# gpcv-liujin/Ada-MVS

Hardware: AMD Instinct MI355X
Metric: depth maps/sec at 768x384x5-view x192-hyp (hot path, features resident in HBM) (higher is better)
Workload: dtype f32; 1 GPU; cfg2: 5 views, 768x384, hypotheses 192, fp32; concurrent_tile_groups=1, parallelism=tile-sharded x1, 1 RCCL gather per step, launch=hipGraph replay

## Files before the change

### ada-mvs_amd/csrc/api.hip

```cpp
#include <stdarg.h>
#include <string.h>

#include <atomic>
#include <mutex>

#include "../../include/adamvs_hip.h"
#include "common.h"
#include "kernels.h"

namespace adamvs {

thread_local char g_last_error[512] = "";

int set_error(int code, const char* fmt, ...) {
  va_list ap;
  va_start(ap, fmt);
  vsnprintf(g_last_error, sizeof(g_last_error), fmt, ap);
  va_end(ap);
  return code;
}

static_assert(sizeof(FuseWeights) == sizeof(adamvs_fuse_weights), "adamvs_fuse_weights layout");

struct OptionEntry { const char* name; int def; };
// ... 86 lines not shown
    size_t F = (size_t)s.S * s.B * hw * stage_reg_width(s);
    c.sim = take(F);
    c.score = take(F);
    c.creg = take(3 * F);
  }
  c.total = o;
  return c;
}

static int check_desc(const adamvs_stage_desc* d) {
  ADAMVS_CHECK_ARG(d, "stage: null descriptor");
  ADAMVS_CHECK_ARG(d->B > 0 && d->S > 0 && d->D > 1 && d->h > 1 && d->w > 1, "stage: bad shape (B=%d S=%d D=%d h=%d w=%d)",
                   d->B, d->S, d->D, d->h, d->w);
  ADAMVS_CHECK_ARG(d->C == 8 || d->C == 16 || d->C == 32, "stage: C=%d unsupported (8, 16 or 32)", d->C);
  ADAMVS_CHECK_ARG((d->h % 2) == 0 && (d->w % 2) == 0, "stage: h=%d w=%d must be even", d->h, d->w);
  ADAMVS_CHECK_ARG(d->B <= 65535, "stage: B=%d tiles per call (at most 65535)", d->B);
  ADAMVS_CHECK_ARG(d->precision == PRECISION_FP32 || d->precision == PRECISION_BF16X3, "stage: precision=%d (0 fp32, 1 bf16x3)", d->precision);
  ADAMVS_CHECK_ARG(d->eps_in_numerator == 0 || d->eps_in_numerator == 1, "stage: eps_in_numerator=%d (0 or 1)", d->eps_in_numerator);
  ADAMVS_CHECK_ARG(d->plane_mode >= PLANES_EXPLICIT && d->plane_mode <= PLANES_WINDOW, "stage: plane_mode=%d (0 explicit, 1 uniform, 2 window)", d->plane_mode);
  ADAMVS_CHECK_ARG(d->precision_fuse == PRECISION_FP32 || d->precision_fuse == PRECISION_BF16X3,
                   "stage: precision_fuse=%d (0 fp32, 1 bf16x3)", d->precision_fuse);
  if (d->first_stage) {
    ADAMVS_CHECK_ARG(stage_reg_width(*d) > 0, "stage: D=%d hypotheses: CostRegNet2D runs at widths up to 512", d->D);
    ADAMVS_CHECK_ARG((d->h % 8) == 0 && (d->w % 8) == 0, "stage: first stage needs h=%d w=%d multiples of 8", d->h, d->w);
  } else {
    ADAMVS_CHECK_ARG(d->prev_h > 0 && d->prev_w > 0, "stage: prev_h/prev_w missing");
  }
  return 0;
}

}

using namespace adamvs;

extern "C" int adamvs_version(void) { return ADAMVS_ABI_VERSION; }

extern "C" int adamvs_option_count(void) { return OPT_COUNT; }
extern "C" const char* adamvs_option_name(int index) { return index >= 0 && index < OPT_COUNT ? g_option_table[index].name : nullptr; }
extern "C" int adamvs_option_default(const char* name, int* value) {
  const int i = option_index(name);
  ADAMVS_CHECK_ARG(i >= 0 && value, "option_default: unknown option '%s' (include/adamvs_hip.h, OPTIONS)", name ? name : "(null)");
  *value = g_option_table[i].def;
  return 0;
}
extern "C" int adamvs_get_option(const char* name, int* value) {
  const int i = option_index(name);
  ADAMVS_CHECK_ARG(i >= 0 && value, "get_option: unknown option '%s' (include/adamvs_hip.h, OPTIONS)", name ? name : "(null)");
  *value = opt((Option)i);
  return 0;
}
extern "C" int adamvs_set_option(const char* name, int value) {
  const int i = option_index(name);
  ADAMVS_CHECK_ARG(i >= 0, "set_option: unknown option '%s' (include/adamvs_hip.h, OPTIONS)", name ? name : "(null)");
  option_init();
  g_option_value[i].store(value, std::memory_order_relaxed);
  return 0;
}
extern "C" const char* adamvs_last_error_string(void) { return g_last_error; }

extern "C" size_t adamvs_slice_reg_step_scratch_bytes(int B, int h, int w) {
  size_t hw = (size_t)h * w, hw4 = (size_t)(h / 2) * (w / 2);
  return (3 * align_up((size_t)B * hw * 8) + 3 * align_up((size_t)B * hw4 * 16)) * sizeof(float);
}

extern "C" int adamvs_slice_reg_step(const float* cost, float* state1, float* state2, const adamvs_fuse_weights* weights,
                                     float* reg_cost, int B, int C, int h, int w, int in_up, int precision, void* scratch,
                                     size_t scratch_bytes, void* stream) {
  ADAMVS_CHECK_ARG(precision == PRECISION_FP32 || precision == PRECISION_BF16X3, "slice_reg_step: precision=%d (0 fp32, 1 bf16x3)", precision);
  ADAMVS_CHECK_ARG(cost && state1 && state2 && weights && reg_cost && scratch, "slice_reg_step: null pointer");
  ADAMVS_CHECK_ARG(B > 0 && h > 1 && w > 1 && (h % 2) == 0 && (w % 2) == 0, "slice_reg_step: bad shape (B=%d h=%d w=%d, even sizes)", B, h, w);
  ADAMVS_CHECK_ARG(C == 8 || C == 16 || C == 32, "slice_reg_step: C=%d unsupported (8, 16 or 32)", C);
  ADAMVS_CHECK_ARG(scratch_bytes >= adamvs_slice_reg_step_scratch_bytes(B, h, w), "slice_reg_step: scratch too small");
  hipStream_t st = (hipStream_t)stream;
  size_t n1 = align_up((size_t)B * h * w * 8), n2 = align_up((size_t)B * (h / 2) * (w / 2) * 16);
  float* s = (float*)scratch;
  float* c1 = s;
  StepBuffers sb{state1, s + n1, s + 2 * n1, s + 3 * n1, state2, s + 3 * n1 + n2, s + 3 * n1 + 2 * n2};
  FuseWeights fw;
  memcpy(&fw, weights, sizeof(fw));
  int rc = launch_conv1(cost, fw.conv1, c1, B, C, h, w, precision, st);
  if (rc) return rc;
  float* h1_now = state1;
  float* h2_now = state2;
  if ((rc = launch_slice_step(c1, fw, sb, reg_cost, B, h, w, 1, 0, in_up, precision, st, &h1_now, &h2_now))) return rc;
  if (h1_now != state1) {
    hipError_t e = copy_floats(h1_now, state1, (size_t)B * h * w * 8, st);
    if (e != hipSuccess) return set_error((int)e, "slice_reg_step: state copy: %s", hipGetErrorString(e));
  }
  if (h2_now != state2) {
    hipError_t e = copy_floats(h2_now, state2, (size_t)B * (h / 2) * (w / 2) * 16, st);
    if (e != hipSuccess) return set_error((int)e, "slice_reg_step: state copy: %s", hipGetErrorString(e));
  }
  return 0;
}

extern "C" int adamvs_recurrence_schedule(int precision_fuse, long long pixels) { return recurrence_mode(precision_fuse, (long)pixels); }
extern "C" int adamvs_gru_wino_mask(void) { return gru_wino_mask(); }

extern "C" size_t adamvs_depth_stage_workspace_bytes(const adamvs_stage_desc* desc) {
  if (check_desc(desc)) return 0;
  return carve(*desc).total * sizeof(float);
}

static int stage_forward(const adamvs_stage_desc* desc, const float* feat, const float* rt, const float* planes,
                         const float* prev_conf, const float* w_reg, size_t w_reg_floats, const adamvs_fuse_weights* w_fuse,
                         float* view_weight, float* pair_depth, float* depth, float* confidence, int phases, void* workspace,
                         size_t workspace_bytes, void* stream, bool timing_only) {
  int rc = check_desc(desc);
  if (rc) return rc;
  ADAMVS_CHECK_ARG(phases >= 0 && phases <= ADAMVS_PHASE_ALL, "stage: phases=%d (a subset of ADAMVS_PHASE_ALL = 15)", phases);
  const adamvs_stage_desc& s = *desc;
  ADAMVS_CHECK_ARG(feat && rt && planes && w_fuse && view_weight && depth && confidence && workspace, "stage: null pointer");
  ADAMVS_CHECK_ARG(!s.first_stage || (w_reg && pair_depth), "stage: first stage needs w_reg and pair_depth");
  ADAMVS_CHECK_ARG(!s.first_stage || w_reg_floats == cost_reg_weight_floats(stage_reg_width(s), s.precision),
                   "stage: w_reg holds %zu floats; D=%d hypotheses run at width %d, whose layout has %zu (include/adamvs_hip.h)",
                   w_reg_floats, s.D, stage_reg_width(s), cost_reg_weight_floats(stage_reg_width(s), s.precision));
  ADAMVS_CHECK_ARG(s.first_stage || prev_conf, "stage: later stages need prev_conf");
  StageCarve c = carve(s);
  ADAMVS_CHECK_ARG(workspace_bytes >= c.total * sizeof(float), "stage: workspace too small (%zu < %zu bytes)", workspace_bytes,
                   c.total * sizeof(float));
  hipStream_t st = (hipStream_t)stream;
  float* ws = (float*)workspace;
  FuseWeights fw;
  memcpy(&fw, w_fuse, sizeof(fw));
  const PlaneSrc ps{planes, s.plane_mode, s.half_span, s.plane_mode == PLANES_WINDOW ? s.half_span_dev : nullptr};

  if (!(phases & ADAMVS_PHASE_VIEW_WEIGHTS)) {
  } else if (s.first_stage) {
    const int Dr = stage_reg_width(s);
    if ((rc = launch_pair_similarity(feat, rt, ps, ws + c.sim, s.B, s.S, s.C, s.D, s.h, s.w, st, Dr))) return rc;
    if (cost_reg_softmax_fusable(Dr, s.precision, ps)) {
      if ((rc = launch_cost_reg_net_2d(ws + c.sim, w_reg, ws + c.creg, ws + c.score, s.S * s.B, Dr, s.h, s.w, s.precision, st,
                                       view_weight, pair_depth, &ps, s.B, s.D)))
        return rc;
    } else {
      if ((rc = launch_cost_reg_net_2d(ws + c.sim, w_reg, ws + c.creg, ws + c.score, s.S * s.B, Dr, s.h, s.w, s.precision, st))) return rc;
      if ((rc = launch_softmax_regress(ws + c.score, ps, view_weight, pair_depth, s.S, s.B, Dr, s.h, s.w, st, s.D))) return rc;
    }
  } else {
    if ((rc = adamvs_resize_bilinear(prev_conf, view_weight, s.S * s.B, s.prev_h, s.prev_w, s.h, s.w, stream))) return rc;
  }

  const bool do_agg = phases & ADAMVS_PHASE_AGGREGATE, do_rec = phases & ADAMVS_PHASE_RECURRENCE, do_arg = phases & ADAMVS_PHASE_SOFT_ARGMIN;
  if (!do_agg && !do_rec && !do_arg) return 0;
  const size_t hw = (size_t)s.h * s.w, hw4 = (size_t)(s.h / 2) * (s.w / 2);
  const int dc = c.dc, nchunks = (s.D + dc - 1) / dc;
  ADAMVS_CHECK_ARG(nchunks == 1 || (do_agg && do_rec && do_arg) || timing_only,
                   "stage: phases=%d selects a proper subset of AGGREGATE|RECURRENCE|SOFT_ARGMIN, but D=%d runs in %d chunks of %d "
                   "hypotheses and the workspace keeps one: pass all three in one call (adamvs_bench_stage_phase times one "
                   "phase alone, no maps)", phases, s.D, nchunks, dc);
  const size_t c1_stride = (size_t)s.B * hw * 8;
  GruStateRing rb{{ws + c.h1[0], ws + c.h1[1], ws + c.h1[2], ws + c.h1[3]}, ws + c.rh1, ws + c.u1, {ws + c.c2[0], ws + c.c2[1]},
                  {ws + c.h2[0], ws + c.h2[1]}, ws + c.rh2, ws + c.u2};
  const int mode = recurrence_mode(s.precision_fuse, (long)s.B * s.h * s.w);
  const bool pipelined = mode != 0;
  const int lag = recurrence_lags(mode, s.precision_fuse).dec;
  if (do_rec) {
    hipError_t e = zero_floats(pipelined ? rb.h1[3] : rb.h1[0], (size_t)s.B * hw * 8, st);
    if (e == hipSuccess) e = zero_floats(pipelined ? rb.h2[1] : rb.h2[0], (size_t)s.B * hw4 * 16, st);
    if (e != hipSuccess) return set_error((int)e, "stage: zero initial states: %s", hipGetErrorString(e));
  }
  auto vol_of = [&](int d) { return ws + c.vol[(d / dc) & 1]; };
  auto argmin_chunk = [&](int k) {
    const int d0 = k * dc, nd = (d0 + dc < s.D ? d0 + dc : s.D) - d0;
    return launch_soft_argmin_chunk(ws + c.vol[k & 1], dc, ps, s.D, d0, nd, ws + c.acc, k == 0, k == nchunks - 1, depth, confidence,
                                    s.B, s.h, s.w, s.in_up, st);
  };
  StepBuffers sb{rb.h1[0], rb.rh1, rb.u1, rb.c2[0], rb.h2[0], rb.rh2, rb.u2};
  for (int k = 0; k < nchunks; ++k) {
    const int d0 = k * dc, d1 = d0 + dc < s.D ? d0 + dc : s.D;
    if (do_agg && (rc = launch_sweep_conv1_chunk(feat, rt, ps, view_weight, fw.conv1, ws + c.c1, ws + c.agg, s.B, s.S, s.C, s.D, d0,
                                                 d1, s.h, s.w, s.precision_fuse, s.eps_in_numerator, st)))
      return rc;
    if (do_rec) {
      for (int t = d0; t < d1; ++t) {
        const float* c1_t = ws + c.c1 + (size_t)(t - d0) * c1_stride;
        if (pipelined) {
          const int sd = t - lag;
          if ((rc = launch_recur_pipeline_step(rb, fw, s.B, s.h, s.w, s.D, t, c1_t, sd >= 0 ? vol_of(sd) : nullptr, dc, sd >= 0 ? sd % dc : 0,
                                               s.in_up, s.precision_fuse, mode, st)))
            return rc;
          if (do_arg && sd >= 0 && sd % dc == dc - 1 && (rc = argmin_chunk(sd / dc))) return rc;
        } else if ((rc = launch_slice_step(c1_t, fw, sb, vol_of(t), s.B, s.h, s.w, dc, t % dc, s.in_up, s.precision_fuse, st))) {
          return rc;
        }
      }
      if (!pipelined && do_arg && (rc = argmin_chunk(k))) return rc;
    } else if (do_arg && (rc = argmin_chunk(k))) {
      return rc;
    }
  }
  if (do_rec && pipelined) {
    for (int t = s.D; t < s.D + lag; ++t) {
      const int sd = t - lag;
      if ((rc = launch_recur_pipeline_step(rb, fw, s.B, s.h, s.w, s.D, t, nullptr, sd >= 0 ? vol_of(sd) : nullptr, dc, sd >= 0 ? sd % dc : 0,
                                           s.in_up, s.precision_fuse, mode, st)))
        return rc;
      if (do_arg && sd >= 0 && sd % dc == dc - 1 && sd / dc < nchunks - 1 && (rc = argmin_chunk(sd / dc))) return rc;
    }
    if (do_arg && (rc = argmin_chunk(nchunks - 1))) return rc;
  }
  return 0;
}

extern "C" int adamvs_depth_stage_forward(const adamvs_stage_desc* desc, const float* feat, const float* rt,
                                          const float* planes, const float* prev_conf, const float* w_reg, size_t w_reg_floats,
                                          const adamvs_fuse_weights* w_fuse, float* view_weight, float* pair_depth,
                                          float* depth, float* confidence, int phases, void* workspace,
                                          size_t workspace_bytes, void* stream) {
  return stage_forward(desc, feat, rt, planes, prev_conf, w_reg, w_reg_floats, w_fuse, view_weight, pair_depth, depth, confidence,
                       phases, workspace, workspace_bytes, stream, false);
}

extern "C" int adamvs_bench_stage_phase(const adamvs_stage_desc* desc, const float* feat, const float* rt,
                                        const float* planes, const float* prev_conf, const float* w_reg, size_t w_reg_floats,
                                        const adamvs_fuse_weights* w_fuse, float* view_weight, float* pair_depth,
                                        float* depth, float* confidence, int phases, void* workspace,
                                        size_t workspace_bytes, void* stream) {
  return stage_forward(desc, feat, rt, planes, prev_conf, w_reg, w_reg_floats, w_fuse, view_weight, pair_depth, depth, confidence,
                       phases, workspace, workspace_bytes, stream, true);
}

extern "C" int adamvs_fusion_max_sources(void) { return ADAMVS_FUSION_MAX_SOURCES; }

static bool finite_f(float v) { return v == v && v <= 3.402823466e38f && v >= -3.402823466e38f; }

extern "C" int adamvs_geo_consistency(const float* ref_depth, const float* ref_conf, int H, int W, const adamvs_fusion_source* sources,
                                      int N, float prob_threshold, float pix_threshold, float rel_depth_threshold, int min_consistent,
                                      unsigned char* count, float* fused, unsigned* block_kept, void* stream) {
  ADAMVS_CHECK_ARG(ref_depth && ref_conf && sources && count && fused && block_kept, "geo_consistency: null pointer");
  ADAMVS_CHECK_ARG(H > 0 && W > 0 && (long)H * W < (1L << 31), "geo_consistency: bad reference size H=%d W=%d", H, W);
  ADAMVS_CHECK_ARG(N >= 1 && N <= ADAMVS_FUSION_MAX_SOURCES, "geo_consistency: N=%d sources (1 .. %d)", N, ADAMVS_FUSION_MAX_SOURCES);
  ADAMVS_CHECK_ARG(finite_f(prob_threshold), "geo_consistency: prob_threshold is not finite");
  ADAMVS_CHECK_ARG(finite_f(pix_threshold) && pix_threshold > 0.f, "geo_consistency: pix_threshold must be finite and > 0");
  ADAMVS_CHECK_ARG(finite_f(rel_depth_threshold) && rel_depth_threshold > 0.f, "geo_consistency: rel_depth_threshold must be finite and > 0");
  ADAMVS_CHECK_ARG(min_consistent >= 0, "geo_consistency: min_consistent=%d (>= 0)", min_consistent);
  for (int s = 0; s < N; ++s) {
    ADAMVS_CHECK_ARG(sources[s].depth, "geo_consistency: source %d: null depth pointer", s);
    ADAMVS_CHECK_ARG(sources[s].H > 0 && sources[s].W > 0 && (long)sources[s].H * sources[s].W < (1L << 31),
                     "geo_consistency: source %d: bad size H=%d W=%d", s, sources[s].H, sources[s].W);
    for (int k = 0; k < 12; ++k)
      ADAMVS_CHECK_ARG(finite_f(sources[s].fwd[k]) && finite_f(sources[s].back[k]), "geo_consistency: source %d: transform not finite", s);
  }
  return launch_geo_consistency(ref_depth, ref_conf, H, W, sources, N, prob_threshold, pix_threshold, rel_depth_threshold, min_consistent,
                                count, fused, block_kept, (hipStream_t)stream);
}

extern "C" int adamvs_fusion_scan(const unsigned* block_kept, unsigned* offsets, int nblocks, void* stream) {
  ADAMVS_CHECK_ARG(block_kept && offsets, "fusion_scan: null pointer");
  ADAMVS_CHECK_ARG(nblocks > 0, "fusion_scan: nblocks=%d (> 0)", nblocks);
  return launch_fusion_scan(block_kept, offsets, nblocks, (hipStream_t)stream);
}

extern "C" int adamvs_fusion_emit(const float* fused, const unsigned char* rgba, int H, int W, const double* camera, const unsigned* offsets,
                                  double* xyz, unsigned char* rgb, long capacity, void* stream) {
  ADAMVS_CHECK_ARG(fused && rgba && camera && offsets && xyz && rgb, "fusion_emit: null pointer");
  ADAMVS_CHECK_ARG(H > 0 && W > 0 && (long)H * W < (1L << 31), "fusion_emit: bad size H=%d W=%d", H, W);
  ADAMVS_CHECK_ARG(capacity >= (long)H * W, "fusion_emit: capacity %ld < H W = %ld points", capacity, (long)H * W);
  for (int k = 0; k < 21; ++k)
    ADAMVS_CHECK_ARG(std::isfinite(camera[k]), "fusion_emit: camera[%d] is not finite", k);
  return launch_fusion_emit(fused, rgba, H, W, camera, offsets, xyz, rgb, capacity, (hipStream_t)stream);
}

static int dsm_check_grid(const adamvs_dsm_grid* g, const char* what) {
  ADAMVS_CHECK_ARG(g, "%s: null grid", what);
  ADAMVS_CHECK_ARG(std::isfinite(g->gsd) && g->gsd > 0.0, "%s: gsd=%g must be finite and > 0", what, g->gsd);
  ADAMVS_CHECK_ARG(std::isfinite(g->x0) && std::isfinite(g->y_top) && std::isfinite(g->z_ref), "%s: grid origin / z_ref not finite", what);
  ADAMVS_CHECK_ARG(g->W > 0 && g->H > 0 && (long)g->W * g->H <= ADAMVS_DSM_MAX_CELLS, "%s: grid W=%d H=%d (W H <= %d cells)", what, g->W,
                   g->H, ADAMVS_DSM_MAX_CELLS);
  return 0;
}

static int dsm_check_points(long n, long seq0, const char* what) {
  ADAMVS_CHECK_ARG(n >= 0, "%s: n=%ld (>= 0)", what, n);
  ADAMVS_CHECK_ARG(seq0 >= 0 && seq0 <= (1L << 32) - n, "%s: seq0=%ld + n=%ld exceeds 2^32 points", what, seq0, n);
  return 0;
}

extern "C" int adamvs_dsm_accumulate(const adamvs_dsm_grid* grid, const double* xyz, long n, long seq0, int mode, unsigned long long* key,
                                     unsigned* count, long long* sum, void* stream) {
  if (int rc = dsm_check_grid(grid, "dsm_accumulate")) return rc;
  if (int rc = dsm_check_points(n, seq0, "dsm_accumulate")) return rc;
  ADAMVS_CHECK_ARG(mode == ADAMVS_DSM_MAX || mode == ADAMVS_DSM_MEAN, "dsm_accumulate: mode=%d (0 max, 1 mean)", mode);
  ADAMVS_CHECK_ARG(xyz && key && count && (sum || mode == ADAMVS_DSM_MAX), "dsm_accumulate: null pointer");
  return launch_dsm_accumulate(*grid, xyz, n, seq0, mode, key, count, sum, (hipStream_t)stream);
}

extern "C" int adamvs_dsm_claim(const adamvs_dsm_grid* grid, const double* xyz, const unsigned char* rgb, long n, long seq0,
                                const unsigned long long* key, unsigned* color, void* stream) {
  if (int rc = dsm_check_grid(grid, "dsm_claim")) return rc;
  if (int rc = dsm_check_points(n, seq0, "dsm_claim")) return rc;
  ADAMVS_CHECK_ARG(xyz && rgb && key && color, "dsm_claim: null pointer");
  return launch_dsm_claim(*grid, xyz, rgb, n, seq0, key, color, (hipStream_t)stream);
}

extern "C" int adamvs_dsm_finalize(const adamvs_dsm_grid* grid, const unsigned long long* key, const unsigned* count, const long long* sum,
                                   const unsigned* color, int mode, int min_count, float* dsm, unsigned short* count16, unsigned char* rgba,
                                   void* stream) {
  if (int rc = dsm_check_grid(grid, "dsm_finalize")) return rc;
  ADAMVS_CHECK_ARG(mode == ADAMVS_DSM_MAX || mode == ADAMVS_DSM_MEAN, "dsm_finalize: mode=%d (0 max, 1 mean)", mode);
  ADAMVS_CHECK_ARG(min_count >= 1, "dsm_finalize: min_count=%d (>= 1)", min_count);
  ADAMVS_CHECK_ARG(key && count && color && dsm && count16 && rgba && (sum || mode == ADAMVS_DSM_MAX), "dsm_finalize: null pointer");
  return launch_dsm_finalize(*grid, key, count, sum, color, mode, min_count, dsm, count16, (unsigned*)rgba, (hipStream_t)stream);
}

static int dsm_fill_check_size(int W, int H, const char* what) {
  ADAMVS_CHECK_ARG(W > 0 && H > 0 && (long)W * H <= ADAMVS_DSM_MAX_CELLS, "%s: grid W=%d H=%d (W H <= %d cells)", what, W, H,
// ... 658 lines not shown
```

### ada-mvs_amd/csrc/kernels.h

```cpp
#pragma once
#include <stdlib.h>

#include "common.h"
#include "options.h"
#include "planes.h"
#include "../../include/adamvs_hip.h"

namespace adamvs {

enum { PRECISION_FP32 = 0, PRECISION_BF16X3 = 1 };

hipError_t zero_floats(float* p, size_t n, hipStream_t st);
hipError_t copy_floats(const float* src, float* dst, size_t n, hipStream_t st);

struct FuseWeights {
  const float* conv1;
  const float* gates1; const float* gates1_b;
  const float* cand1;  const float* cand1_b;
  const float* conv2;
  const float* gates2; const float* gates2_b;
  const float* cand2;  const float* cand2_b;
  const float* upconv1; const float* upconv1_b;
  const float* final_w;
  const float* gates1_w; const float* gates2_w; const float* cand2_w; const float* cand1_w;
};
int gru_wino_mask();

struct StepBuffers {
  float* h1; float* rh1; float* u1;
  float* c2; float* h2; float* rh2; float* u2;
};

struct GruStateRing {
  float* h1[4]; float* rh1; float* u1;
  float* c2[2]; float* h2[2]; float* rh2; float* u2;
};
struct RecurLags { int c2, dec; };
int recurrence_mode(int precision, long pixels);
RecurLags recurrence_lags(int schedule, int precision);
int launch_recur_pipeline_step(const GruStateRing& rb, const FuseWeights& fw, int B, int h, int w, int D, int t, const float* c1_t,
                               float* vol_dec, int D_vol, int d_dec, int in_up, int precision, int schedule, hipStream_t st);
int launch_soft_argmin_chunk(const float* vol, int vol_D, PlaneSrc planes, int D, int d0, int nd, float* acc, int first, int last,
                             float* depth, float* conf, int B, int h, int w, int in_up, hipStream_t st);
int sweep_chunk_planes(int D);
int launch_sweep_conv1_chunk(const float* feat, const float* rt, PlaneSrc planes, const float* vw, const float* w1pk,
                             float* c1_chunk, float* sim_ws, int B, int S, int C, int D, int d0, int d1, int h, int w, int precision,
                             int eps_in_numerator, hipStream_t st);

int launch_conv1(const float* cost, const float* w, float* c1, int B, int C, int h, int w_, int precision, hipStream_t st);
int launch_conv1_bf16x3(const float* cost, const float* w, float* c1, int N, int C, int h, int w_, hipStream_t st);
int launch_gru_convs_bf16x3(const float* c1, const FuseWeights& fw, const StepBuffers& sb, int B, int h, int w, int d,
                            float** h1_now, float** h2_now, hipStream_t st);
int launch_slice_step(const float* c1, const FuseWeights& fw, const StepBuffers& sb, float* vol, int B, int h, int w, int D,
                      int d, int in_up, int precision, hipStream_t st, float** h1_now = nullptr, float** h2_now = nullptr);
enum { GRU_PRO_NONE = 0, GRU_PRO_GATES = 1, GRU_PRO_OUT = 2 };
struct GruPro {
  int mode;
  const float* f;
  const float* o;
  const double* part_f;
  const double* part_o;
  int parts_f, group_f, parts_o;
  const float* gn_f;
  const float* gn_o;
  float* state_out;
  float* R; int RW;
  int hc, count;
  float eps;
};

constexpr int GN_PARTS_LIMIT = 2048;
inline bool gn_epilogue_partials(long parts, int samples) { return parts > 0 && parts <= GN_PARTS_LIMIT && parts * samples <= 4096; }
int launch_conv_pair(const float* srcA, int CA, const float* srcB, int CB, const float* wpk, const float* bias, float* out,
                     int cout, int B, int h, int w, hipStream_t st, double* gn_part = nullptr, int gn_hc = 0, int gn_groups = 0,
                     int* gn_parts = nullptr, const GruPro* pro = nullptr);
bool conv_pair_epilogue_partials(int B, int h, int w);
inline bool gru_fold_enabled(int samples) {
  const int forced = opt(OPT_RED_FOLD_APPLIES);
  return forced >= 0 ? forced != 0 : samples <= 2;
}
bool can_fold_gru_applies(int N, int D, int h, int w);
int launch_conv_dd_gates_gn(const float* in, const float* wpk_r, const float* bias_r, const float* skip_r, float* out_r,
                            const float* wpk_u, const float* bias_u, const float* skip_u, float* out_u, int N, int D, int h, int w,
                            hipStream_t st, double* gn_part, int gn_n, int* gn_parts, const GruPro* pro = nullptr);
int launch_conv_dd_gn(const float* in, const float* wpk, const float* bias, const float* skip, float* out, int N, int D, int h, int w,
                      hipStream_t st, double* gn_part, int gn_n, int gn_group, int gn_ngroups, int* gn_parts, const GruPro* pro = nullptr);
int launch_soft_argmin(const float* vol, const float* planes, float* depth, float* conf, int B, int D, int h, int w,
                       int in_up, hipStream_t st);
int launch_sweep_conv1(const float* feat, const float* rt, PlaneSrc planes, const float* vw, const float* w1pk,
                       float* c1, float* sim_ws, int B, int S, int C, int D, int h, int w, int precision, int eps_in_numerator,
                       hipStream_t st);
int launch_sweep_variance(const float* feat, const float* rt, const float* planes, float* out_a, int Da, float* out_b, int Db,
                          int B, int S, int C, int D, int h, int w, hipStream_t st);
size_t sweep_workspace_floats(int B, int C, int D, int h, int w);
int launch_cost_reg_net_2d(const float* x, const float* wpk, float* ws, float* score, int N, int D, int h, int w,
                           int precision, hipStream_t st, float* sm_vw = nullptr, float* sm_pd = nullptr,
                           const PlaneSrc* sm_planes = nullptr, int sm_B = 1, int n_planes = 0);
size_t cost_reg_weight_floats(int D, int precision);
int costreg_width(int D);
int costreg_width_bf16x3(int D);
bool cost_reg_softmax_fusable(int D, int precision, const PlaneSrc& planes);
int launch_conv_dd_bf16x3(const float* in, const float* wpk, const float* bias, const float* skip, float* out, int N, int D,
                          int hi, int wi, int ho, int wo, int mode, int relu, hipStream_t st, float* sm_vw = nullptr,
                          float* sm_pd = nullptr, const PlaneSrc* sm_planes = nullptr, int sm_B = 1, int n_planes = 0);
bool costreg_bf16x3_depth_supported(int D);
bool wino_depth_supported(int D);
bool cost_reg_winograd(int D, int precision);
bool wino_softmax_fused();
size_t wino_softmax_part_floats(int N, int D, int h, int w);
int launch_conv_wino_softmax(const float* in, const float* wpk, const float* bias, float* part, const PlaneSrc& planes, float* vw, float* pd,
                             int N, int B, int D, int n_planes, int h, int w, hipStream_t st);
int launch_conv_wino(const float* in, const float* wpk, const float* bias, const float* skip, float* out, int N, int D, int h, int w,
                     int relu, hipStream_t st);

int launch_pair_similarity(const float* feat, const float* rt, PlaneSrc planes, float* sim, int B, int S, int C, int D, int h,
                           int w, hipStream_t st, int Dw = 0);
int launch_softmax_regress(const float* score, PlaneSrc planes, float* vw, float* pd, int S, int B, int D, int h, int w,
                           hipStream_t st, int n_planes = 0);
bool costreg_depth_supported(int D);

constexpr int FUSION_TILE = ADAMVS_FUSION_TILE;
constexpr int FUSION_MAX_SOURCES = ADAMVS_FUSION_MAX_SOURCES;
int launch_geo_consistency(const float* ref_depth, const float* ref_conf, int H, int W, const adamvs_fusion_source* srcs, int N,
                           float prob_threshold, float pix_threshold, float rel_depth_threshold, int min_consistent, uint8_t* count,
                           float* fused, unsigned* block_kept, hipStream_t st);
int launch_fusion_scan(const unsigned* counts, unsigned* offsets, int nblocks, hipStream_t st);
int launch_fusion_emit(const float* fused, const uint8_t* rgba, int H, int W, const double* camera, const unsigned* offsets, double* xyz,
                       uint8_t* rgb, long capacity, hipStream_t st);

constexpr int DSM_TILE = 256;
int launch_dsm_accumulate(const adamvs_dsm_grid& g, const double* xyz, long n, long seq0, int mode, unsigned long long* key,
                          unsigned* count, long long* sum, hipStream_t st);
int launch_dsm_claim(const adamvs_dsm_grid& g, const double* xyz, const uint8_t* rgb, long n, long seq0, const unsigned long long* key,
                     unsigned* color, hipStream_t st);
int launch_dsm_finalize(const adamvs_dsm_grid& g, const unsigned long long* key, const unsigned* count, const long long* sum,
                        const unsigned* color, int mode, int min_count, float* dsm, uint16_t* count16, unsigned* rgba, hipStream_t st);

long dsm_fill_workspace_bytes(int W, int H);
int launch_dsm_fill(int W, int H, const float* dsm, const uint8_t* rgba, double r_cells, double tol_height, double tol_colour,
                    int max_cycles, void* workspace, float* dsm_out, uint8_t* rgba_out, int* dist2, uint8_t* filled,
                    adamvs_dsm_fill_stats* stats, hipStream_t st);

constexpr int MESH_TILE = ADAMVS_MESH_TILE;
int launch_tsdf_integrate(const adamvs_mesh_brick& b, const adamvs_mesh_view* views, int nviews, const int* list, int nlist, float* tsdf,
                          uint16_t* weight, unsigned* rgba, hipStream_t st);
int launch_mesh_classify(const adamvs_mesh_brick& b, const float* tsdf, const uint16_t* weight, unsigned* cube_code, unsigned* block_tris,
                         hipStream_t st);
int launch_mesh_count_vertices(const adamvs_mesh_brick& b, const float* tsdf, const unsigned* cube_code, uint8_t* edge_mask,
                               unsigned* block_verts, hipStream_t st);
int launch_mesh_emit(const adamvs_mesh_brick& b, const float* tsdf, const unsigned* rgba, const unsigned* cube_code, const uint8_t* edge_mask,
                     const unsigned* vert_offsets, const unsigned* tri_offsets, unsigned vertex_base, double* xyz, uint8_t* rgb,
                     unsigned* first_vertex, long vert_capacity, unsigned* faces, long tri_capacity, hipStream_t st);

constexpr int SIMPLIFY_TILE = ADAMVS_SIMPLIFY_TILE;
int launch_simplify_keys(const double* origin, double cell, const double* xyz, long nv, long long* keys, uint8_t* bad, hipStream_t st);
int launch_simplify_corners(const unsigned* faces, long nf, const int* vcell, long nv, int nc, int* fcell, int* entry_cell, uint8_t* survive,
                            hipStream_t st);
int launch_simplify_accumulate(const double* origin, double cell, const long long* keys, int nc, const double* xyz, const uint8_t* rgb,
                               long nv, const unsigned* faces, long nf, const long long* entry, const long long* fstart,
                               const long long* vorder, const long long* vstart, double* quadric, double* member,
                               unsigned long long* colour, hipStream_t st);
int launch_simplify_solve(const double* origin, double cell, double rank_eps, const long long* keys, int nc, const double* quadric,
                          const double* member, const unsigned long long* colour, const long long* vstart, double* pos, uint8_t* col,
                          uint8_t* rank, uint8_t* fallback, double* error, hipStream_t st);
void simplify_solve_host(const double* quadric, const double* mean, double cell, double rank_eps, double* p, int* rank, int* fallback,
                         double* error);
int launch_simplify_triples(const int* fcell, long nf, const long long* surv, long ns, int* tri, hipStream_t st);
int launch_simplify_first(const int* tri, const long long* surv, const long long* order, long ns, long nf, uint8_t* keep, hipStream_t st);
int launch_simplify_mark(const int* fcell, const uint8_t* keep, long nf, int nc, uint8_t* used, hipStream_t st);
int launch_simplify_count(const uint8_t* flags, long n, unsigned* block_count, hipStream_t st);
int launch_simplify_emit(const double* pos, const uint8_t* col, const uint8_t* used, int nc, const unsigned* cell_offsets, const int* fcell,
                         const uint8_t* keep, long nf, const unsigned* face_offsets, double* xyz, uint8_t* rgb, unsigned* new_index,
                         long vert_capacity, unsigned* faces, long face_capacity, hipStream_t st);

constexpr int SMOOTH_TILE = ADAMVS_SMOOTH_TILE;
int launch_smooth_faces(const double* p, long nv, const unsigned* faces, long nf, double* rec, hipStream_t st);
int launch_mesh_edge_keys(const unsigned* faces, long nf, long long* keys, const char* what, hipStream_t st);
int launch_smooth_boundary(const long long* keys, long n, long nv, uint8_t* fixed, hipStream_t st);
int launch_smooth_filter(const double* rec, const double* nin, double* nout, const unsigned* faces, long nf, long nv, const int* vface,
                         const long long* vstart, double sigma_s, double sigma_r, hipStream_t st);
int launch_smooth_centroids(const double* p, long nv, const unsigned* faces, long nf, double* cen, hipStream_t st);
int launch_smooth_update(const double* p0, const double* p, double* pout, long nv, const double* nrm, const double* cen, long nf,
                         const int* vface, const long long* vstart, const uint8_t* fixed, double cap, uint8_t* clamped, hipStream_t st);

constexpr int CLEAN_TILE = ADAMVS_CLEAN_TILE;
constexpr int CLEAN_CHUNK = ADAMVS_CLEAN_CHUNK;
int launch_clean_components(const unsigned* faces, long nf, long nv, const int* parent_in, int* parent_out, unsigned* changed, hipStream_t st);
int launch_clean_area(const double* area, long nf, const long long* order, const long long* seg_of, const long long* seg_start, long ncomp,
                      double* lead, double* first, double* out, hipStream_t st);
int launch_clean_boundary(const long long* keys, const long long* entry, long n, uint8_t* bnd, hipStream_t st);
int launch_clean_successor(const unsigned* faces, long ns, long nv, const uint8_t* bnd, int* out_cnt, int* in_cnt, int* out_he, int* succ,
                           int* lab, int* nxt, uint8_t* broken, hipStream_t st);
int launch_clean_double(const uint8_t* bnd, long n, const int* lab_in, const int* nxt_in, const uint8_t* broken_in, int* lab_out, int* nxt_out,
                        uint8_t* broken_out, hipStream_t st);
// ... 76 lines not shown
```

### ada-mvs_amd/csrc/options.h

```cpp
#pragma once

namespace adamvs {

#define ADAMVS_OPTION_LIST(X)                                                                                                     \
  X(OPT_WINOGRAD, "winograd", 1)                      \
  X(OPT_WINO_SOFTMAX, "wino_softmax", 1)                              \
  X(OPT_WINO_WPS, "wino_wps", 0)                                                   \
  X(OPT_FUSE_SOFTMAX, "fuse_softmax", 1)                        \
  X(OPT_S2_PAIRS, "s2_pairs", 1)                            \
  X(OPT_CONV_ROWS2, "conv_rows2", -1)                               \
  X(OPT_T2_FUSED, "t2_fused", -1)                                  \
  X(OPT_T2_KB8, "t2_kb8", 1)                                                 \
  X(OPT_COSTREG_DEFER_SKIPS, "costreg_defer_skips", 1)                            \
  X(OPT_CONV256_SPLIT, "conv256_split", 1)                                          \
  X(OPT_CONV_SMALL_GRID, "conv_small_grid", 1024)         \
  X(OPT_RED_FOLD_APPLIES, "red_fold_applies", -1)               \
  X(OPT_CONV1_F23, "conv1_f23", 3)                             \
  X(OPT_FCONV_F23, "fconv_f23", 1)                                \
  X(OPT_GRU_WINO, "gru_wino", 7)                      \
  X(OPT_RECUR_MODE, "recur_mode", -1)

enum Option {
#define ADAMVS_OPTION_ENUM(e, n, d) e,
  ADAMVS_OPTION_LIST(ADAMVS_OPTION_ENUM)
#undef ADAMVS_OPTION_ENUM
  OPT_COUNT
};

int opt(Option o);

}
```

### ada-mvs_amd/csrc/recurrence.hip

```cpp
#include <stdlib.h>

#include "common.h"
#include "kernels.h"
#include "persistent.h"
#include "slice_roles.h"
#include "slice_roles_bx3.h"
#include "slice_roles_fused.h"
#include "slice_roles_wino.h"

namespace adamvs {

struct NopRole {
  struct Args {};
  static constexpr size_t LDS_BYTES = 0;
  static int tiles_x(const Args&) { return 1; }
  static int tiles_y(const Args&) { return 1; }
  static __device__ __forceinline__ void run(const Args&, const TileGrid&, TileRange, int, int, float*) {}
};

template <class R0, class R1, class R2>
struct SlotArgs {
  typename R0::Args a0; TileGrid g0; TileRange r0; int n0;
  typename R1::Args a1; TileGrid g1; TileRange r1; int n1;
  typename R2::Args a2; TileGrid g2; TileRange r2;
};

template <class R> struct min_blocks { static constexpr int value = 1; };
template <> struct min_blocks<Gru1FusedBx3Role> { static constexpr int value = 2; };
template <> struct min_blocks<Gru2FusedBx3Role> { static constexpr int value = 2; };
template <> struct min_blocks<Gru2FusedRole<4>> { static constexpr int value = 2; };
template <> struct min_blocks<ConvWinoRole<16, 16, 2, EPI_GATES>> { static constexpr int value = 2; };
constexpr int imax3(int a, int b, int c) { return a > b ? (a > c ? a : c) : (b > c ? b : c); }

template <class R0, class R1, class R2>
__global__ __launch_bounds__(256, imax3(min_blocks<R0>::value, min_blocks<R1>::value, min_blocks<R2>::value)) void k_slot(SlotArgs<R0, R1, R2> s) {
  extern __shared__ __attribute__((aligned(16))) float lds[];
  const int wg = blockIdx.x;
  if (wg < s.n0) R0::run(s.a0, s.g0, s.r0, wg, s.n0, lds);
  else if (wg < s.n0 + s.n1) R1::run(s.a1, s.g1, s.r1, wg - s.n0, s.n1, lds);
  else R2::run(s.a2, s.g2, s.r2, wg - s.n0 - s.n1, (int)gridDim.x - s.n0 - s.n1, lds);
}

constexpr size_t max3(size_t a, size_t b, size_t c) { return a > b ? (a > c ? a : c) : (b > c ? b : c); }

template <class R>
struct RoleUse {
  const typename R::Args* args;
  float cost;
  float f0, f1;
};

template <int NR>
static void split_grid(int total, const long (&tiles)[NR], const double (&work)[NR], int (&n)[NR]) {
  double W = 0;
  for (int i = 0; i < NR; ++i) W += tiles[i] ? work[i] : 0;
  int sum = 0;
  for (int i = 0; i < NR; ++i) {
    n[i] = 0;
    if (!tiles[i]) continue;
    long v = (long)(total * (work[i] / W) + 0.5);
    n[i] = (int)(v < 1 ? 1 : (v > tiles[i] ? tiles[i] : v));
    sum += n[i];
  }
  while (sum > total) {
    int k = -1;
    for (int i = 0; i < NR; ++i) if (n[i] > 1 && (k < 0 || n[i] > n[k])) k = i;
    if (k < 0) break;
    --n[k]; --sum;
  }
  while (sum < total) {
    int k = -1;
    for (int i = 0; i < NR; ++i)
      if (tiles[i] && n[i] < tiles[i] && (k < 0 || work[i] / n[i] > work[k] / n[k])) k = i;
    if (k < 0) break;
    ++n[k]; ++sum;
  }
}

template <class R0, class R1, class R2>
static int launch_slot(const RoleUse<R0>& u0, const RoleUse<R1>& u1, const RoleUse<R2>& u2, int B, hipStream_t st, const char* name) {
  constexpr size_t lds = max3(R0::LDS_BYTES, R1::LDS_BYTES, R2::LDS_BYTES);
  static_assert(lds <= 160 * 1024, "slot exceeds the LDS of a CU");
  constexpr auto kern = k_slot<R0, R1, R2>;
  int capacity, rc;
  if ((rc = resident_capacity<kern>(lds, name, &capacity))) return rc;
  SlotArgs<R0, R1, R2> s;
  memset(&s, 0, sizeof(s));
  long tiles[3] = {0, 0, 0};
  double work[3] = {0, 0, 0};
  auto prep = [&](auto* args, auto& dst_args, TileGrid& g, TileRange& r, float cost, float f0, float f1, int i, auto role) -> int {
    typedef decltype(role) R;
    if (!args) return 0;
    dst_args = *args;
    if (int e = make_tile_grid(g, R::tiles_x(*args), R::tiles_y(*args), B)) return e;
    r.begin = (int)((double)g.ntiles * f0 + 0.5);
    r.end = f1 >= 1.0f ? g.ntiles : (int)((double)g.ntiles * f1 + 0.5);
    tiles[i] = r.end - r.begin;
    work[i] = (double)tiles[i] * cost;
    return 0;
  };
  if ((rc = prep(u0.args, s.a0, s.g0, s.r0, u0.cost, u0.f0, u0.f1, 0, R0()))) return rc;
  if ((rc = prep(u1.args, s.a1, s.g1, s.r1, u1.cost, u1.f0, u1.f1, 1, R1()))) return rc;
  if ((rc = prep(u2.args, s.a2, s.g2, s.r2, u2.cost, u2.f0, u2.f1, 2, R2()))) return rc;
  const long all = tiles[0] + tiles[1] + tiles[2];
  if (all == 0) return 0;
  int n[3];
  split_grid<3>((int)(all < capacity ? all : capacity), tiles, work, n);
  s.n0 = n[0];
  s.n1 = n[1];
  hipLaunchKernelGGL(kern, dim3(n[0] + n[1] + n[2]), dim3(256), lds, st, s);
  ADAMVS_CHECK_LAUNCH(name);
  return 0;
}

template <class R0, class R1, class R2, class R3>
struct SlotArgs4 {
  typename R0::Args a0; TileGrid g0; TileRange r0; int n0;
  typename R1::Args a1; TileGrid g1; TileRange r1; int n1;
  typename R2::Args a2; TileGrid g2; TileRange r2; int n2;
  typename R3::Args a3; TileGrid g3; TileRange r3;
};
constexpr int imax4(int a, int b, int c, int d) { return imax3(imax3(a, b, c), d, d); }
constexpr size_t max4(size_t a, size_t b, size_t c, size_t d) { return max3(max3(a, b, c), d, d); }

template <class R0, class R1, class R2, class R3>
__global__ __launch_bounds__(256, imax4(min_blocks<R0>::value, min_blocks<R1>::value, min_blocks<R2>::value, min_blocks<R3>::value))
void k_slot4(SlotArgs4<R0, R1, R2, R3> s) {
  extern __shared__ __attribute__((aligned(16))) float lds[];
  const int wg = blockIdx.x;
  if (wg < s.n0) R0::run(s.a0, s.g0, s.r0, wg, s.n0, lds);
  else if (wg < s.n0 + s.n1) R1::run(s.a1, s.g1, s.r1, wg - s.n0, s.n1, lds);
  else if (wg < s.n0 + s.n1 + s.n2) R2::run(s.a2, s.g2, s.r2, wg - s.n0 - s.n1, s.n2, lds);
  else R3::run(s.a3, s.g3, s.r3, wg - s.n0 - s.n1 - s.n2, (int)gridDim.x - s.n0 - s.n1 - s.n2, lds);
}

template <class R0, class R1, class R2, class R3>
static int launch_slot4(const RoleUse<R0>& u0, const RoleUse<R1>& u1, const RoleUse<R2>& u2, const RoleUse<R3>& u3, int B, hipStream_t st,
                        const char* name) {
  constexpr size_t lds = max4(R0::LDS_BYTES, R1::LDS_BYTES, R2::LDS_BYTES, R3::LDS_BYTES);
  static_assert(lds <= 64 * 1024, "slot exceeds the default dynamic LDS limit");
  constexpr auto kern = k_slot4<R0, R1, R2, R3>;
  int capacity, rc;
  if ((rc = resident_capacity<kern>(lds, name, &capacity))) return rc;
  SlotArgs4<R0, R1, R2, R3> s;
  memset(&s, 0, sizeof(s));
  long tiles[4] = {0, 0, 0, 0};
  double work[4] = {0, 0, 0, 0};
  auto prep = [&](auto* args, auto& dst_args, TileGrid& g, TileRange& r, float cost, float f0, float f1, int i, auto role) -> int {
    typedef decltype(role) R;
    if (!args) return 0;
    dst_args = *args;
    if (int e = make_tile_grid(g, R::tiles_x(*args), R::tiles_y(*args), B)) return e;
    r.begin = (int)((double)g.ntiles * f0 + 0.5);
    r.end = f1 >= 1.0f ? g.ntiles : (int)((double)g.ntiles * f1 + 0.5);
    tiles[i] = r.end - r.begin;
    work[i] = (double)tiles[i] * cost;
    return 0;
  };
  if ((rc = prep(u0.args, s.a0, s.g0, s.r0, u0.cost, u0.f0, u0.f1, 0, R0()))) return rc;
  if ((rc = prep(u1.args, s.a1, s.g1, s.r1, u1.cost, u1.f0, u1.f1, 1, R1()))) return rc;
  if ((rc = prep(u2.args, s.a2, s.g2, s.r2, u2.cost, u2.f0, u2.f1, 2, R2()))) return rc;
  if ((rc = prep(u3.args, s.a3, s.g3, s.r3, u3.cost, u3.f0, u3.f1, 3, R3()))) return rc;
  const long all = tiles[0] + tiles[1] + tiles[2] + tiles[3];
  if (all == 0) return 0;
  int n[4];
  split_grid<4>((int)(all < capacity ? all : capacity), tiles, work, n);
  s.n0 = n[0]; s.n1 = n[1]; s.n2 = n[2];
  hipLaunchKernelGGL(kern, dim3(n[0] + n[1] + n[2] + n[3]), dim3(256), lds, st, s);
  ADAMVS_CHECK_LAUNCH(name);
  return 0;
}

typedef ConvSmallRole<8, 8, 1, 1, EPI_GATES> Gates1;
typedef Cand1TwoRowRole Cand1;
typedef ConvSmallRole<8, 0, 1, 2, EPI_RELU> Conv2;
typedef ConvSmallRole<16, 16, 2, 1, EPI_GATES> Gates2;
typedef ConvSmallRole<16, 16, 1, 1, EPI_CAND> Cand2;
typedef ConvWinoRole<8, 8, 1, EPI_GATES> Gates1W;
typedef ConvWinoRole<16, 16, 2, EPI_GATES> Gates2W;
typedef ConvWinoRole<16, 16, 1, EPI_CAND> Cand2W;
typedef Gru1FusedRole<4, 2> Gru1S;
typedef Gru2FusedRole<4> Gru2S;
typedef Gru1FusedBx3Role Gru1Bx;
typedef ConvSmallBx3Role<8, 0, 1, 2, BXE_RELU> Conv2Bx;
typedef Gru2FusedBx3Role Gru2Bx;

struct RoleCosts { float g1, c1, v2, g2, c2, dec, k1bx, v2bx, g2bx, c2bx, fa, fb, fd; };
struct FusedCosts { float k1s, k1l, k2s; };
static const FusedCosts& fused_costs() {
  static const FusedCosts c = [] {
    FusedCosts v = {10.0f, 23.0f, 15.0f};
    if (const char* e = getenv("ADAMVS_RECUR_COSTS_FUSED")) {
      float a, b, d;
      if (sscanf(e, "%f,%f,%f", &a, &b, &d) == 3 && a > 0.f && b > 0.f && d > 0.f && a < 1e6f && b < 1e6f && d < 1e6f) v = FusedCosts{a, b, d};
      else fprintf(stderr, "adamvs: ADAMVS_RECUR_COSTS_FUSED ignored (three positive values)\n");
    }
    return v;
  }();
  return c;
}
static RoleCosts parse_role_costs() {
  RoleCosts c = {2.85f, 4.07f, 2.39f, 9.98f, 5.53f, 5.0f, 11.3f, 3.2f, 12.0f, 5.0f, 0.6f, 0.8f, 0.42f};
  if (const char* e = getenv("ADAMVS_RECUR_COSTS")) {
    float v[13];
    bool ok = sscanf(e, "%f,%f,%f,%f,%f,%f,%f,%f,%f,%f,%f,%f,%f", v, v + 1, v + 2, v + 3, v + 4, v + 5, v + 6, v + 7, v + 8, v + 9, v + 10,
                     v + 11, v + 12) == 13;
    for (int i = 0; ok && i < 10; ++i) ok = v[i] > 0.f && v[i] < 1e6f;
    for (int i = 10; ok && i < 13; ++i) ok = v[i] >= 0.f && v[i] <= 1.f;
    if (ok) c = RoleCosts{v[0], v[1], v[2], v[3], v[4], v[5], v[6], v[7], v[8], v[9], v[10], v[11], v[12]};
    else fprintf(stderr, "adamvs: ADAMVS_RECUR_COSTS ignored (13 comma-separated values: 10 positive costs, 3 fractions in [0,1])\n");
  }
  return c;
}
static const RoleCosts& role_costs() {
  static const RoleCosts c = parse_role_costs();
  return c;
}

int recurrence_mode(int precision, long pixels) {
  const int forced = opt(OPT_RECUR_MODE);
  if (forced == 0 || forced == 1 || forced == 3 || forced == 5) return forced;
  if (precision != PRECISION_FP32) return pixels <= 250000 ? 5 : (pixels <= 1000000 ? 3 : 0);
  return pixels <= 100000 ? 5 : (pixels <= 200000 ? 3 : (pixels <= 800000 ? 1 : 0));
}

template <class R> static RoleUse<R> use(const typename R::Args* a, float cost, float f0 = 0.f, float f1 = 1.f) {
  return RoleUse<R>{a, cost, f0, f1};
}
template <class R> static RoleUse<R> none() { return RoleUse<R>{nullptr, 0.f, 0.f, 1.f}; }

RecurLags recurrence_lags(int schedule, int precision) {
  if (schedule == 5) return RecurLags{2, 3};
  return RecurLags{1, 2};
}

int launch_recur_pipeline_step(const GruStateRing& rb, const FuseWeights& fw, int B, int h, int w, int D, int t, const float* c1_t,
                               float* vol_dec, int D_vol, int d_dec, int in_up, int precision, int schedule, hipStream_t st) {
  const int h2 = h / 2, w2 = w / 2;
  const RecurLags lag = recurrence_lags(schedule, precision);
  const int s2 = t - 1, sc = t - lag.c2, sd = t - lag.dec;
  const bool l1 = t < D, l2 = s2 >= 0 && s2 < D, lc = sc >= 0 && sc < D, dec = sd >= 0 && sd < D;
  auto H1 = [&](int s) { return rb.h1[((s % 4) + 4) % 4]; };
  auto H2 = [&](int s) { return rb.h2[((s % 2) + 2) % 2]; };
  auto C2 = [&](int s) { return rb.c2[((s % 2) + 2) % 2]; };
  const RoleCosts& k = role_costs();
  int rc;
  DecoderArgs da{H2(sd), H1(sd), fw.upconv1, fw.upconv1_b, fw.final_w, vol_dec, h, w, D_vol, d_dec};

  if (precision == PRECISION_BF16X3) {
    Gru1Args g1{c1_t, H1(t - 1), H1(t), (const bf16x8*)fw.gates1, fw.gates1_b, (const bf16x8*)fw.cand1, fw.cand1_b, h, w};
    SmallConvArgsBx v2{H1(s2), nullptr, (const bf16x8*)fw.conv2, nullptr, C2(s2), nullptr, nullptr, h, w, h2, w2, 16, nullptr};
    if (schedule == 5) {
      Gru2Args g2s{C2(sc), H2(sc - 1), H2(sc), (const bf16x8*)fw.gates2, fw.gates2_b, (const bf16x8*)fw.cand2, fw.cand2_b, h2, w2};
      if (in_up)
        return launch_slot4<Gru1Bx, Conv2Bx, Gru2Bx, DecoderRole<true>>(
            l1 ? use<Gru1Bx>(&g1, k.k1bx) : none<Gru1Bx>(), l2 ? use<Conv2Bx>(&v2, k.v2bx) : none<Conv2Bx>(), lc ? use<Gru2Bx>(&g2s, k.g2bx) : none<Gru2Bx>(),
            dec ? use<DecoderRole<true>>(&da, k.dec) : none<DecoderRole<true>>(), B, st, "recurrence, one launch (bf16x3)");
      return launch_slot4<Gru1Bx, Conv2Bx, Gru2Bx, DecoderRole<false>>(
          l1 ? use<Gru1Bx>(&g1, k.k1bx) : none<Gru1Bx>(), l2 ? use<Conv2Bx>(&v2, k.v2bx) : none<Conv2Bx>(), lc ? use<Gru2Bx>(&g2s, k.g2bx) : none<Gru2Bx>(),
          dec ? use<DecoderRole<false>>(&da, k.dec) : none<DecoderRole<false>>(), B, st, "recurrence, one launch (bf16x3)");
    }
    Gru2Args g2{C2(s2), H2(s2 - 1), H2(s2), (const bf16x8*)fw.gates2, fw.gates2_b, (const bf16x8*)fw.cand2, fw.cand2_b, h2, w2};
    float f = 0.5f + ((0.54f * k.g2bx + 1.0f * k.dec) - 0.94f * k.v2bx) / (2.f * k.k1bx);
    f = !l2 ? 1.0f : (f < 0.1f ? 0.1f : (f > 1.f ? 1.f : f));
    if (l1 || l2)
      if ((rc = launch_slot<Gru1Bx, Conv2Bx, NopRole>(l1 ? use<Gru1Bx>(&g1, k.k1bx, 0.f, f) : none<Gru1Bx>(),
                                                      l2 ? use<Conv2Bx>(&v2, k.v2bx) : none<Conv2Bx>(), none<NopRole>(), B, st,
                                                      "recurrence slot A (bf16x3)")))
        return rc;
    const bool rest = l1 && f < 1.f;
    if (!(rest || l2 || dec)) return 0;
    if (in_up)
      return launch_slot<Gru1Bx, Gru2Bx, DecoderRole<true>>(rest ? use<Gru1Bx>(&g1, k.k1bx, f, 1.f) : none<Gru1Bx>(),
                                                            l2 ? use<Gru2Bx>(&g2, k.g2bx) : none<Gru2Bx>(),
                                                            dec ? use<DecoderRole<true>>(&da, k.dec) : none<DecoderRole<true>>(), B, st,
                                                            "recurrence slot B (bf16x3)");
    return launch_slot<Gru1Bx, Gru2Bx, DecoderRole<false>>(rest ? use<Gru1Bx>(&g1, k.k1bx, f, 1.f) : none<Gru1Bx>(),
                                                           l2 ? use<Gru2Bx>(&g2, k.g2bx) : none<Gru2Bx>(),
                                                           dec ? use<DecoderRole<false>>(&da, k.dec) : none<DecoderRole<false>>(), B, st,
                                                           "recurrence slot B (bf16x3)");
  }

  if (schedule == 5) {
    const FusedCosts& fk = fused_costs();
    Gru1F32Args f1{c1_t, H1(t - 1), H1(t), fw.gates1, fw.gates1_b, fw.cand1, fw.cand1_b, h, w};
    SmallConvArgs v2s{H1(s2), nullptr, fw.conv2, nullptr, C2(s2), nullptr, h, w, h2, w2, 16, nullptr};
    Gru2F32Args f2{C2(sc), H2(sc - 1), H2(sc), fw.gates2, fw.gates2_b, fw.cand2, fw.cand2_b, h2, w2};
    if (in_up)
      return launch_slot4<Gru1S, Conv2, Gru2S, DecoderRole<true>>(
          l1 ? use<Gru1S>(&f1, fk.k1s) : none<Gru1S>(), l2 ? use<Conv2>(&v2s, k.v2) : none<Conv2>(), lc ? use<Gru2S>(&f2, fk.k2s) : none<Gru2S>(),
          dec ? use<DecoderRole<true>>(&da, k.dec) : none<DecoderRole<true>>(), B, st, "recurrence, one launch (fp32)");
    return launch_slot4<Gru1S, Conv2, Gru2S, DecoderRole<false>>(
        l1 ? use<Gru1S>(&f1, fk.k1s) : none<Gru1S>(), l2 ? use<Conv2>(&v2s, k.v2) : none<Conv2>(), lc ? use<Gru2S>(&f2, fk.k2s) : none<Gru2S>(),
        dec ? use<DecoderRole<false>>(&da, k.dec) : none<DecoderRole<false>>(), B, st, "recurrence, one launch (fp32)");
  }
  SmallConvArgs g1{c1_t, H1(t - 1), fw.gates1, fw.gates1_b, rb.rh1, rb.u1, h, w, h, w, 16, nullptr};
  SmallConvArgs c1{c1_t, rb.rh1, fw.cand1, fw.cand1_b, H1(t), rb.u1, h, w, h, w, 8, H1(t - 1)};
  SmallConvArgs v2{H1(s2), nullptr, fw.conv2, nullptr, C2(s2), nullptr, h, w, h2, w2, 16, nullptr};
  SmallConvArgs g2{C2(s2), H2(s2 - 1), fw.gates2, fw.gates2_b, rb.rh2, rb.u2, h2, w2, h2, w2, 32, nullptr};
  SmallConvArgs c2{C2(sc), rb.rh2, fw.cand2, fw.cand2_b, H2(sc), rb.u2, h2, w2, h2, w2, 16, H2(sc - 1)};
  if (schedule == 3) {
    Conv2Gates2Args vg{H1(s2), H2(s2 - 1), fw.conv2, fw.gates2, fw.gates2_b, C2(s2), rb.rh2, rb.u2, h, w, h2, w2};
    if (l1 || l2)
      if ((rc = launch_slot<Gates1, Conv2Gates2Role<0>, Conv2Gates2Role<1>>(
               l1 ? use<Gates1>(&g1, k.g1) : none<Gates1>(), l2 ? use<Conv2Gates2Role<0>>(&vg, 0.5f * k.g2 + k.v2) : none<Conv2Gates2Role<0>>(),
               l2 ? use<Conv2Gates2Role<1>>(&vg, 0.5f * k.g2 + k.v2) : none<Conv2Gates2Role<1>>(), B, st, "recurrence slot A (schedule 3)")))
        return rc;
    if (!(l1 || lc || dec)) return 0;
    if (in_up)
      return launch_slot<Cand1, Cand2, DecoderRole<true>>(l1 ? use<Cand1>(&c1, k.c1) : none<Cand1>(), lc ? use<Cand2>(&c2, k.c2) : none<Cand2>(),
                                                          dec ? use<DecoderRole<true>>(&da, k.dec) : none<DecoderRole<true>>(), B, st,
                                                          "recurrence slot B (schedule 3)");
    return launch_slot<Cand1, Cand2, DecoderRole<false>>(l1 ? use<Cand1>(&c1, k.c1) : none<Cand1>(), lc ? use<Cand2>(&c2, k.c2) : none<Cand2>(),
                                                         dec ? use<DecoderRole<false>>(&da, k.dec) : none<DecoderRole<false>>(), B, st,
                                                         "recurrence slot B (schedule 3)");
  }
  if (schedule == 1 && (gru_wino_mask() & 7) == 7 && fw.gates1_w && fw.gates2_w && fw.cand2_w) {
    SmallConvArgs g1w = g1, g2w = g2, c2w = c2;
    g1w.wpk = fw.gates1_w; g2w.wpk = fw.gates2_w; c2w.wpk = fw.cand2_w;
    const float kg1 = 4.f * 0.76f * k.g1, kg2 = 4.f * 0.69f * k.g2, kc2 = 4.f * 0.89f * k.c2;
    if (l1 || l2)
      if ((rc = launch_slot<Gates1W, Conv2, NopRole>(l1 ? use<Gates1W>(&g1w, kg1) : none<Gates1W>(), l2 ? use<Conv2>(&v2, k.v2) : none<Conv2>(),
                                                     none<NopRole>(), B, st, "recurrence slot A (F(2x2,3x3))")))
        return rc;
    if (l1 || l2)
      if ((rc = launch_slot<Cand1, Gates2W, NopRole>(l1 ? use<Cand1>(&c1, k.c1) : none<Cand1>(), l2 ? use<Gates2W>(&g2w, kg2) : none<Gates2W>(),
                                                     none<NopRole>(), B, st, "recurrence slot B (F(2x2,3x3))")))
        return rc;
    if (lc || dec) {
      if (in_up)
        rc = launch_slot<Cand2W, DecoderRole<true>, NopRole>(lc ? use<Cand2W>(&c2w, kc2) : none<Cand2W>(),
                                                             dec ? use<DecoderRole<true>>(&da, k.dec) : none<DecoderRole<true>>(),
                                                             none<NopRole>(), B, st, "recurrence slot C (F(2x2,3x3))");
      else
        rc = launch_slot<Cand2W, DecoderRole<false>, NopRole>(lc ? use<Cand2W>(&c2w, kc2) : none<Cand2W>(),
                                                              dec ? use<DecoderRole<false>>(&da, k.dec) : none<DecoderRole<false>>(),
                                                              none<NopRole>(), B, st, "recurrence slot C (F(2x2,3x3))");
      if (rc) return rc;
    }
    return 0;
  }
  if (l1 || l2)
    if ((rc = launch_slot<Gates1, Conv2, NopRole>(l1 ? use<Gates1>(&g1, k.g1) : none<Gates1>(), l2 ? use<Conv2>(&v2, k.v2) : none<Conv2>(),
                                                  none<NopRole>(), B, st, "recurrence slot A")))
      return rc;
  if (l1 || l2)
    if ((rc = launch_slot<Cand1, Gates2, NopRole>(l1 ? use<Cand1>(&c1, k.c1) : none<Cand1>(), l2 ? use<Gates2>(&g2, k.g2) : none<Gates2>(),
                                                  none<NopRole>(), B, st, "recurrence slot B")))
      return rc;
  if (lc || dec) {
    if (in_up)
      rc = launch_slot<Cand2, DecoderRole<true>, NopRole>(lc ? use<Cand2>(&c2, k.c2) : none<Cand2>(),
                                                          dec ? use<DecoderRole<true>>(&da, k.dec) : none<DecoderRole<true>>(),
                                                          none<NopRole>(), B, st, "recurrence slot C");
    else
      rc = launch_slot<Cand2, DecoderRole<false>, NopRole>(lc ? use<Cand2>(&c2, k.c2) : none<Cand2>(),
                                                           dec ? use<DecoderRole<false>>(&da, k.dec) : none<DecoderRole<false>>(),
                                                           none<NopRole>(), B, st, "recurrence slot C");
    if (rc) return rc;
  }
  return 0;
}

template <bool IN_UP>
__global__ void k_soft_argmin_chunk(const float* __restrict__ vol, int vol_D, PlaneSrc planes, int D, int d0, int nd,
                                    float* __restrict__ acc, int first, int last, float* __restrict__ depth,
                                    float* __restrict__ conf, int h, int w, size_t total) {
  size_t i = (size_t)blockIdx.x * blockDim.x + threadIdx.x;
  if (i >= total) return;
  const int Ho = IN_UP ? 2 * h : h, Wo = IN_UP ? 2 * w : w;
  int X = (int)(i % Wo), Y = (int)((i / Wo) % Ho);
  size_t b = i / ((size_t)Wo * Ho);
  size_t hw = (size_t)h * w, HW = (size_t)Ho * Wo;
  int y0 = Y, y1 = Y, x0 = X, x1 = X; float ly = 0.f, lx = 0.f;
  if (IN_UP) {
    float sy = fmaxf(((float)Y + 0.5f) * 0.5f - 0.5f, 0.f), sx = fmaxf(((float)X + 0.5f) * 0.5f - 0.5f, 0.f);
    y0 = (int)sy; x0 = (int)sx;
    y1 = y0 + (y0 < h - 1 ? 1 : 0); x1 = x0 + (x0 < w - 1 ? 1 : 0);
    ly = sy - (float)y0; lx = sx - (float)x0;
  }
  const float* v = vol + b * vol_D * HW + (size_t)Y * Wo + X;
  const PlaneLine p00 = plane_line(planes, b, (size_t)y0 * w + x0, D, hw), p01 = plane_line(planes, b, (size_t)y0 * w + x1, D, hw);
  const PlaneLine p10 = plane_line(planes, b, (size_t)y1 * w + x0, D, hw), p11 = plane_line(planes, b, (size_t)y1 * w + x1, D, hw);
  float E = 0.f, M = 0.f, A = 0.f;
  if (!first) { E = acc[i]; M = acc[total + i]; A = acc[2 * total + i]; }
#pragma unroll 8
  for (int d = 0; d < nd; ++d) {
    float pr = __expf(v[(size_t)d * HW]);
    float dep;
    if (IN_UP) {
      float top = plane_at(planes, p00, d0 + d, hw) * (1.f - lx) + plane_at(planes, p01, d0 + d, hw) * lx;
      float bot = plane_at(planes, p10, d0 + d, hw) * (1.f - lx) + plane_at(planes, p11, d0 + d, hw) * lx;
      dep = top * (1.f - ly) + bot * ly;
    } else {
      dep = plane_at(planes, p00, d0 + d, hw);
    }
    M = (M < pr) ? pr : M;
    A = dep * pr + A;
    E = E + pr;
  }
  if (last) {
    float den = E + 1e-10f;
    depth[i] = A / den;
    conf[i] = M / den;
  } else {
    acc[i] = E; acc[total + i] = M; acc[2 * total + i] = A;
  }
}

int launch_soft_argmin_chunk(const float* vol, int vol_D, PlaneSrc planes, int D, int d0, int nd, float* acc, int first, int last,
                             float* depth, float* conf, int B, int h, int w, int in_up, hipStream_t st) {
  size_t total = (size_t)B * (in_up ? 4 : 1) * h * w;
  unsigned nb = (unsigned)((total + 255) / 256);
  if (in_up)
    hipLaunchKernelGGL((k_soft_argmin_chunk<true>), dim3(nb), dim3(256), 0, st, vol, vol_D, planes, D, d0, nd, acc, first, last, depth,
                       conf, h, w, total);
  else
    hipLaunchKernelGGL((k_soft_argmin_chunk<false>), dim3(nb), dim3(256), 0, st, vol, vol_D, planes, D, d0, nd, acc, first, last, depth,
                       conf, h, w, total);
  ADAMVS_CHECK_LAUNCH("soft_argmin (chunk)");
  return 0;
}

}
```

### ada-mvs_amd/csrc/slice_red.hip

```cpp
#include "common.h"
#include "conv_frag.h"
#include "kernels.h"
#include "persistent.h"
#include "slice_roles.h"
#include "slice_roles_wino.h"

namespace adamvs {

template <int CA, int CB, int NT, int EPI>
__global__ __launch_bounds__(256, 2) void k_conv_small_wino(SmallConvArgs a, TileGrid tg) {
  extern __shared__ __attribute__((aligned(16))) float lds[];
  ConvWinoRole<CA, CB, NT, EPI>::run(a, tg, TileRange{0, tg.ntiles}, blockIdx.x, gridDim.x, lds);
}

template <int CA, int CB, int NT, int STRIDE, int EPI, int TR, int RW>
__global__ __launch_bounds__(256) void k_conv_small(SmallConvArgs a, TileGrid tg) {
  extern __shared__ __attribute__((aligned(16))) float lds[];
  ConvSmallRole<CA, CB, NT, STRIDE, EPI, TR, RW>::run(a, tg, TileRange{0, tg.ntiles}, blockIdx.x, gridDim.x, lds);
}
template <int CA, int CB, int NT>
__global__ __launch_bounds__(256) void k_conv_small_pro(SmallConvArgs a, TileGrid tg, GruPro pro) {
  extern __shared__ __attribute__((aligned(16))) float lds[];
  ConvSmallRole<CA, CB, NT, 1, EPI_LINEAR, 4, 1>::run(a, tg, TileRange{0, tg.ntiles}, blockIdx.x, gridDim.x, lds, pro);
}

#ifndef DEC_WAVES
#define DEC_WAVES 4
#endif
template <bool IN_UP>
__global__ __launch_bounds__(256, DEC_WAVES) void k_decoder(DecoderArgs a, TileGrid tg) {
  extern __shared__ __attribute__((aligned(16))) float lds[];
  DecoderRole<IN_UP>::run(a, tg, TileRange{0, tg.ntiles}, blockIdx.x, gridDim.x, lds);
}

__global__ __launch_bounds__(256) void k_cand1_two_row(SmallConvArgs a, TileGrid tg) {
  extern __shared__ __attribute__((aligned(16))) float lds[];
  Cand1TwoRowRole::run(a, tg, TileRange{0, tg.ntiles}, blockIdx.x, gridDim.x, lds);
}


template <bool IN_UP>
__global__ void k_soft_argmin(const float* __restrict__ vol, const float* __restrict__ planes, float* __restrict__ depth,
                              float* __restrict__ conf, int D, int h, int w, size_t total) {
  size_t i = (size_t)blockIdx.x * blockDim.x + threadIdx.x;
  if (i >= total) return;
  const int Ho = IN_UP ? 2 * h : h, Wo = IN_UP ? 2 * w : w;
  int X = (int)(i % Wo), Y = (int)((i / Wo) % Ho);
  size_t b = i / ((size_t)Wo * Ho);
  size_t hw = (size_t)h * w, HW = (size_t)Ho * Wo;
  int y0 = Y, y1 = Y, x0 = X, x1 = X; float ly = 0.f, lx = 0.f;
  if (IN_UP) {
    float sy = fmaxf(((float)Y + 0.5f) * 0.5f - 0.5f, 0.f), sx = fmaxf(((float)X + 0.5f) * 0.5f - 0.5f, 0.f);
    y0 = (int)sy; x0 = (int)sx;
    y1 = y0 + (y0 < h - 1 ? 1 : 0); x1 = x0 + (x0 < w - 1 ? 1 : 0);
    ly = sy - (float)y0; lx = sx - (float)x0;
  }
  const float* v = vol + b * D * HW + (size_t)Y * Wo + X;
  const float* pl = planes + b * D * hw;
  float E = 0.f, M = 0.f, A = 0.f;
  for (int d = 0; d < D; ++d) {
    float pr = __expf(v[(size_t)d * HW]);
    const float* q = pl + (size_t)d * hw;
    float dep;
    if (IN_UP) {
      float top = q[y0 * w + x0] * (1.f - lx) + q[y0 * w + x1] * lx;
      float bot = q[y1 * w + x0] * (1.f - lx) + q[y1 * w + x1] * lx;
      dep = top * (1.f - ly) + bot * ly;
    } else {
      dep = q[y0 * w + x0];
    }
    M = (M < pr) ? pr : M;
    A = dep * pr + A;
    E = E + pr;
  }
  float den = E + 1e-10f;
  depth[i] = A / den;
  conf[i] = M / den;
}


template <int CA, int CB, int NT, int STRIDE, int EPI, int TR, int RW>
static int launch_small_shape(const SmallConvArgs& a, int B, hipStream_t st, const char* name) {
  constexpr int TC = 16 * RW;
  constexpr int LR = (STRIDE == 1) ? TR + 2 : 2 * TR + 1;
  constexpr int LC = (STRIDE == 1) ? TC + 2 : 2 * TC + 1;
  constexpr int PLANE = (STRIDE == 1) ? plane_pitch16(LR * LC) : ((LR * LC) | 1);
  constexpr size_t lds = (size_t)((CA + CB) / 4) * group_pitch(PLANE, (CA + CB) / 4) * sizeof(float);
  static_assert(lds <= 64 * 1024, "tile exceeds the default dynamic LDS limit");
  TileGrid tg;
  if (int rc = make_tile_grid(tg, cdiv(a.wo, TC), cdiv(a.ho, TR), B)) return rc;
  return launch_resident<k_conv_small<CA, CB, NT, STRIDE, EPI, TR, RW>>(tg.ntiles, lds, st, name, a, tg);
}

template <int CA, int CB, int NT, int EPI>
static int launch_small_wino(const SmallConvArgs& a, int B, hipStream_t st, const char* name) {
  typedef ConvWinoRole<CA, CB, NT, EPI> Role;
  TileGrid tg;
  if (int rc = make_tile_grid(tg, Role::tiles_x(a), Role::tiles_y(a), B)) return rc;
  return launch_resident<k_conv_small_wino<CA, CB, NT, EPI>>(tg.ntiles, Role::LDS_BYTES, st, name, a, tg);
}

int gru_wino_mask() { return opt(OPT_GRU_WINO); }

template <int CA, int CB, int NT, int STRIDE, int EPI>
static int launch_small(const SmallConvArgs& a, int B, hipStream_t st, const char* name) {
  return launch_small_shape<CA, CB, NT, STRIDE, EPI, 4, 1>(a, B, st, name);
}

template <int C>
__global__ __launch_bounds__(256) void k_conv1_two_row(const float* __restrict__ src, const float* __restrict__ wpk,
                                                       float* __restrict__ c1, int h, int w, TileGrid tg) {
  constexpr int KC = C / 4, G = C / 4, TR = 8, TC = 16, LR = TR + 2, LC = TC + 2, NPIX = LR * LC;
  constexpr int PLANE = plane_pitch16(NPIX), GP = group_pitch(PLANE, G);
  constexpr int NL = (NPIX * G + 255) / 256;
  extern __shared__ float lds[];
  const int tid = threadIdx.x, lane = tid & 63, wave = __builtin_amdgcn_readfirstlane(tid >> 6);
  const int p = lane & 15, q = lane >> 4;
  float wf[12][KC];
#pragma unroll
  for (int t = 0; t < 12; ++t)
#pragma unroll
    for (int kc = 0; kc < KC; ++kc) wf[t][kc] = wpk[(t * KC + kc) * 64 + lane];

  unsigned goff[NL], lbyte[NL];
  int rc[NL];
#pragma unroll
  for (int k = 0; k < NL; ++k) {
    const int j = min(tid + k * 256, NPIX * G - 1);
    const int g = j % G, pp = j / G, r = pp / LC, c = pp % LC;
    goff[k] = (unsigned)(((r * w + c) * C + 4 * g) * 4);
    lbyte[k] = (unsigned)((g * GP + r * LC + c) * 4);
    rc[k] = r | (c << 16);
    pin(goff[k]); pin(lbyte[k]); pin(rc[k]);
  }
  unsigned xbyte[KC];
#pragma unroll
  for (int kc = 0; kc < KC; ++kc) {
    xbyte[kc] = (unsigned)((kc * GP + q * PLANE + (2 * wave) * LC + p) * 4);
    pin(xbyte[kc]);
  }
  const int orow = 2 * wave + (q >> 1);
  unsigned ooff = (unsigned)(((orow * w + p) * 8 + 4 * (q & 1)) * 4);
  pin(ooff);

  auto load_tile = [&](f32x4 (&stage)[NL], int n, int tx, int ty) {
    const int ix0 = tx * TC - 1, iy0 = ty * TR - 1;
    const buf_rsrc rs = make_rsrc((const char*)src + (((long)n * h + iy0) * w + ix0) * (C * 4));
    if (iy0 >= 0 && ix0 >= 0 && iy0 + LR <= h && ix0 + LC <= w) {
#pragma unroll
      for (int k = 0; k < NL; ++k) stage[k] = buf_load4(rs, goff[k]);
    } else {
#pragma unroll
      for (int k = 0; k < NL; ++k) {
        const int iy = iy0 + (rc[k] & 0xffff), ix = ix0 + (rc[k] >> 16);
        stage[k] = buf_load4(rs, ((unsigned)iy < (unsigned)h && (unsigned)ix < (unsigned)w) ? goff[k] : BUF_OOB);
      }
    }
  };
  auto store_tile = [&](const f32x4 (&stage)[NL]) {
#pragma unroll
    for (int k = 0; k < NL; ++k) {
      float* dl = (float*)((char*)lds + lbyte[k]);
      f32x4 v = stage[k];
      dl[0] = v.x; dl[PLANE] = v.y; dl[2 * PLANE] = v.z; dl[3 * PLANE] = v.w;
    }
  };

  int t = blockIdx.x;
  if (t >= tg.ntiles) return;
  int n, tx, ty;
  tile_coords(tg, t, n, tx, ty);
  f32x4 stage[NL];
  load_tile(stage, n, tx, ty);
  wait_vmem_all();
  store_tile(stage);
  __syncthreads();
  for (;;) {
    const int tn = t + gridDim.x;
    const bool more = tn < tg.ntiles;
    int nn = 0, txn = 0, tyn = 0;
    if (more) {
      tile_coords(tg, tn, nn, txn, tyn);
      load_tile(stage, nn, txn, tyn);
    }
    f32x4 acc = {0.f, 0.f, 0.f, 0.f};
#pragma unroll
    for (int rr = 0; rr < 4; ++rr)
#pragma unroll
      for (int kx = 0; kx < 3; ++kx)
#pragma unroll
        for (int kc = 0; kc < KC; ++kc)
          acc = mfma16(wf[rr * 3 + kx][kc], *(const float*)((const char*)lds + xbyte[kc] + (rr * LC + kx) * 4), acc);
    drain(acc);

    wait_vmem_all();
    __syncthreads();
    if (more) store_tile(stage);

    const int y0 = ty * TR, x0 = tx * TC;
    const buf_rsrc ro = make_rsrc((char*)c1 + (((long)n * h + y0) * w + x0) * 32);
    unsigned oo = ooff;
    if (!(y0 + TR <= h && x0 + TC <= w)) oo = (y0 + orow < h && x0 + p < w) ? ooff : BUF_OOB;
    acc.x = fmaxf(acc.x, 0.f); acc.y = fmaxf(acc.y, 0.f); acc.z = fmaxf(acc.z, 0.f); acc.w = fmaxf(acc.w, 0.f);
    buf_store4(ro, oo, acc);
    if (!more) break;
    __syncthreads();
    t = tn; n = nn; tx = txn; ty = tyn;
  }
}


static int launch_cand1_two_row(const SmallConvArgs& a, int B, hipStream_t st) {
  constexpr int G = 4;
  constexpr size_t lds = (size_t)G * group_pitch(plane_pitch16(10 * 18), G) * sizeof(float);
  TileGrid tg;
  if (int rc = make_tile_grid(tg, cdiv(a.wo, 16), cdiv(a.ho, 8), B)) return rc;
  return launch_resident<k_cand1_two_row>(tg.ntiles, lds, st, "cand1 (two-row)", a, tg);
}

template <int C>
__global__ __launch_bounds__(256, 3) void k_conv1_ksplit(const float* __restrict__ src, const float* __restrict__ wpk,
                                                      float* __restrict__ c1, int h, int w, TileGrid tg) {
  static_assert(C == 32, "four waves x two k-chunks");
  constexpr int KC = C / 4, G = C / 4, KW = KC / 4, TR = 8, TC = 16, LR = TR + 2, LC = TC + 2, NPIX = LR * LC;
  constexpr int PLANE = plane_pitch16(NPIX), GP = group_pitch(PLANE, G);
  constexpr int NL = (NPIX * G + 255) / 256;
  extern __shared__ __attribute__((aligned(16))) float lds[];
  float* red = lds + G * GP;
  const int tid = threadIdx.x, lane = tid & 63, wave = __builtin_amdgcn_readfirstlane(tid >> 6);
  const int p = lane & 15, q = lane >> 4;
  float wf[12][KW];
#pragma unroll
  for (int t = 0; t < 12; ++t)
#pragma unroll
    for (int kc = 0; kc < KW; ++kc) wf[t][kc] = wpk[(t * KC + wave * KW + kc) * 64 + lane];

  unsigned goff[NL], lbyte[NL];
  int rc[NL];
#pragma unroll
  for (int k = 0; k < NL; ++k) {
    const int j = min(tid + k * 256, NPIX * G - 1);
    const int g = j % G, pp = j / G, r = pp / LC, c = pp % LC;
    goff[k] = (unsigned)(((r * w + c) * C + 4 * g) * 4);
    lbyte[k] = (unsigned)((g * GP + r * LC + c) * 4);
    rc[k] = r | (c << 16);
    pin(goff[k]); pin(lbyte[k]); pin(rc[k]);
  }
  unsigned xbyte[KW];
#pragma unroll
  for (int kc = 0; kc < KW; ++kc) {
    xbyte[kc] = (unsigned)(((wave * KW + kc) * GP + q * PLANE + p) * 4);
    pin(xbyte[kc]);
  }
  unsigned wbyte = (unsigned)(((wave * 3) * 64 + lane) * 16);
  unsigned rbyte[3];
#pragma unroll
  for (int i = 0; i < 3; ++i) {
    const int s = i < wave ? i : i + 1;
    rbyte[i] = (unsigned)(((s * 3 + (wave > s ? wave - 1 : wave)) * 64 + lane) * 16);
    pin(rbyte[i]);
  }
  pin(wbyte);
  const int orow = 2 * wave + (q >> 1);
  unsigned ooff = (unsigned)(((orow * w + p) * 8 + 4 * (q & 1)) * 4);
  pin(ooff);

  auto load_tile = [&](f32x4 (&stage)[NL], int n, int tx, int ty) {
    const int ix0 = tx * TC - 1, iy0 = ty * TR - 1;
    const buf_rsrc rs = make_rsrc((const char*)src + (((long)n * h + iy0) * w + ix0) * (C * 4));
    if (iy0 >= 0 && ix0 >= 0 && iy0 + LR <= h && ix0 + LC <= w) {
#pragma unroll
      for (int k = 0; k < NL; ++k) stage[k] = buf_load4(rs, goff[k]);
    } else {
#pragma unroll
      for (int k = 0; k < NL; ++k) {
        const int iy = iy0 + (rc[k] & 0xffff), ix = ix0 + (rc[k] >> 16);
        stage[k] = buf_load4(rs, ((unsigned)iy < (unsigned)h && (unsigned)ix < (unsigned)w) ? goff[k] : BUF_OOB);
      }
    }
  };
  auto store_tile = [&](const f32x4 (&stage)[NL]) {
#pragma unroll
    for (int k = 0; k < NL; ++k) {
      float* dl = (float*)((char*)lds + lbyte[k]);
      f32x4 v = stage[k];
      dl[0] = v.x; dl[PLANE] = v.y; dl[2 * PLANE] = v.z; dl[3 * PLANE] = v.w;
    }
  };

  int t = blockIdx.x;
  if (t >= tg.ntiles) return;
  int n, tx, ty;
  tile_coords(tg, t, n, tx, ty);
  f32x4 stage[NL];
  load_tile(stage, n, tx, ty);
  wait_vmem_all();
  store_tile(stage);
  __syncthreads();
  for (;;) {
    const int tn = t + gridDim.x;
    const bool more = tn < tg.ntiles;
    int nn = 0, txn = 0, tyn = 0;
    if (more) {
      tile_coords(tg, tn, nn, txn, tyn);
      load_tile(stage, nn, txn, tyn);
    }
    f32x4 acc[4];
#pragma unroll
    for (int rp = 0; rp < 4; ++rp) acc[rp] = f32x4{0.f, 0.f, 0.f, 0.f};
#pragma unroll
    for (int rr = 0; rr < 4; ++rr)
#pragma unroll
      for (int kx = 0; kx < 3; ++kx)
#pragma unroll
        for (int kc = 0; kc < KW; ++kc)
#pragma unroll
          for (int rp = 0; rp < 4; ++rp)
            acc[rp] = mfma16(wf[rr * 3 + kx][kc],
                             *(const float*)((const char*)lds + xbyte[kc] + ((2 * rp + rr) * LC + kx) * 4), acc[rp]);
#pragma unroll
    for (int rp = 0; rp < 4; ++rp)
      if (rp != wave) *(f32x4*)((char*)red + wbyte + (rp > wave ? rp - 1 : rp) * 1024) = acc[rp];

    wait_vmem_all();
    __syncthreads();
    if (more) store_tile(stage);

    f32x4 own = wave == 0 ? acc[0] : (wave == 1 ? acc[1] : (wave == 2 ? acc[2] : acc[3]));
    f32x4 part[3];
#pragma unroll
    for (int i = 0; i < 3; ++i) part[i] = *(const f32x4*)((const char*)red + rbyte[i]);
    f32x4 sum;
    if (wave == 0) sum = ((own + part[0]) + part[1]) + part[2];
    else if (wave == 1) sum = ((part[0] + own) + part[1]) + part[2];
    else if (wave == 2) sum = ((part[0] + part[1]) + own) + part[2];
    else sum = ((part[0] + part[1]) + part[2]) + own;

    const int y0 = ty * TR, x0 = tx * TC;
    const buf_rsrc ro = make_rsrc((char*)c1 + (((long)n * h + y0) * w + x0) * 32);
    unsigned oo = ooff;
    if (!(y0 + TR <= h && x0 + TC <= w)) oo = (y0 + orow < h && x0 + p < w) ? ooff : BUF_OOB;
    sum.x = fmaxf(sum.x, 0.f); sum.y = fmaxf(sum.y, 0.f); sum.z = fmaxf(sum.z, 0.f); sum.w = fmaxf(sum.w, 0.f);
    buf_store4(ro, oo, sum);
    if (!more) break;
    __syncthreads();
    t = tn; n = nn; tx = txn; ty = tyn;
  }
}

template <int C>
__global__ __launch_bounds__(256, 2) void k_conv1_f23(const float* __restrict__ src, const float* __restrict__ wpk,
                                                   float* __restrict__ c1, int h, int w, TileGrid tg) {
  static_assert(C == 32, "two halves of four k-chunks");
  typedef float f32x2c __attribute__((ext_vector_type(2)));
  constexpr int KC = C / 4, G = C / 4, KH = KC / 2, TR = 8, TC = 32, LR = TR + 2, LC = TC + 2, NPIX = LR * LC;
  constexpr int PLANE = plane_pitch16(NPIX), GP = group_pitch(PLANE, G);
  static_assert((PLANE % 2) == 0 && (GP % 2) == 0 && (LC % 2) == 0, "8-byte aligned patch reads");
  constexpr int NL = (NPIX * G + 255) / 256;
  extern __shared__ __attribute__((aligned(16))) float lds[];
  f32x4* red = (f32x4*)(lds + G * GP);
  const int tid = threadIdx.x, lane = tid & 63, wave = __builtin_amdgcn_readfirstlane(tid >> 6);
  const int p = lane & 15, q = lane >> 4;
  const int kh = wave & 1, rp2 = wave >> 1;
  const f32x2c pm = {1.0f, -1.0f};

// ... 184 lines not shown
    }
  };
  auto store_tile = [&](const f32x4 (&stage)[NL]) {
#pragma unroll
    for (int k = 0; k < NL; ++k) {
      float* dl = (float*)((char*)lds + lbyte[k]);
      f32x4 v = stage[k];
      dl[0] = v.x; dl[PLANE] = v.y; dl[2 * PLANE] = v.z; dl[3 * PLANE] = v.w;
    }
  };

  int t = blockIdx.x;
  if (t >= tg.ntiles) return;
  int n, tx, ty;
  tile_coords(tg, t, n, tx, ty);
  f32x4 stage[NL];
  load_tile(stage, n, tx, ty);
  wait_vmem_all();
  store_tile(stage);
  __syncthreads();
  for (;;) {
    const int tn = t + gridDim.x;
    const bool more = tn < tg.ntiles;
    int nn = 0, txn = 0, tyn = 0;
    if (more) {
      tile_coords(tg, tn, nn, txn, tyn);
      load_tile(stage, nn, txn, tyn);
    }
    f32x4 m[4];
#pragma unroll
    for (int j = 0; j < 4; ++j) m[j] = f32x4{0.f, 0.f, 0.f, 0.f};
#pragma unroll
    for (int rr = 0; rr < 4; ++rr)
#pragma unroll
      for (int kc = 0; kc < KC; ++kc) {
        const char* at = (const char*)lds + xb + (kc * GP + rr * LC) * 4;
        const f32x2c d01 = *(const f32x2c*)at, d23 = *(const f32x2c*)(at + 8);
        const f32x2c v03 = d01 - d23;
        const f32x2c v12 = __builtin_elementwise_fma(__builtin_shufflevector(d01, d01, 1, 1), pm, __builtin_shufflevector(d23, d23, 0, 0));
        m[0] = mfma16(uf[rr][0][kc], v03.x, m[0]);
        m[1] = mfma16(uf[rr][1][kc], v12.x, m[1]);
        m[2] = mfma16(uf[rr][2][kc], v12.y, m[2]);
        m[3] = mfma16(uf[rr][3][kc], v03.y, m[3]);
      }
#pragma unroll
    for (int j = 0; j < 4; ++j) drain(m[j]);
    f32x4 o0 = (m[0] + m[1]) + m[2], o1 = (m[1] - m[2]) - m[3];

    wait_vmem_all();
    __syncthreads();
    if (more) store_tile(stage);

    const int y0 = ty * TR, x0 = tx * TC;
    const buf_rsrc ro = make_rsrc((char*)c1 + (((long)n * h + y0) * w + x0) * 32);
    unsigned oa = ooff, ob = ooff + 32;
    if (!(y0 + TR <= h && x0 + TC <= w)) {
      const bool rowok = y0 + orow < h;
      oa = (rowok && x0 + 2 * p < w) ? ooff : BUF_OOB;
      ob = (rowok && x0 + 2 * p + 1 < w) ? ooff + 32 : BUF_OOB;
    }
    o0.x = fmaxf(o0.x, 0.f); o0.y = fmaxf(o0.y, 0.f); o0.z = fmaxf(o0.z, 0.f); o0.w = fmaxf(o0.w, 0.f);
    o1.x = fmaxf(o1.x, 0.f); o1.y = fmaxf(o1.y, 0.f); o1.z = fmaxf(o1.z, 0.f); o1.w = fmaxf(o1.w, 0.f);
    buf_store4(ro, oa, o0);
    buf_store4(ro, ob, o1);
    if (!more) break;
    __syncthreads();
    t = tn; n = nn; tx = txn; ty = tyn;
  }
}

template <int C>
static int launch_conv1_f23_rows(const float* cost, const float* w, float* c1, int N, int h, int w_, hipStream_t st) {
  constexpr int G = C / 4;
  constexpr size_t lds = (size_t)G * ((group_pitch(plane_pitch16(10 * 34), G) + 1) & ~1) * sizeof(float);
  TileGrid tg;
  if (int rc = make_tile_grid(tg, cdiv(w_, 32), cdiv(h, 8), N)) return rc;
  return launch_resident<k_conv1_f23_rows<C>>(tg.ntiles, lds, st, "conv1 (F(2,3) along x)", cost, w, c1, h, w_, tg);
}

static int conv1_f23() { return opt(OPT_CONV1_F23); }

static int launch_conv1_f23_32(const float* cost, const float* w, float* c1, int N, int h, int w_, hipStream_t st) {
  constexpr int C = 32;
  constexpr size_t lds = ((size_t)(C / 4) * group_pitch(plane_pitch16(10 * 34), C / 4) + 4 * 2 * 64 * 4) * sizeof(float);
  static_assert(lds <= 64 * 1024, "default dynamic LDS limit");
  TileGrid tg;
  if (int rc = make_tile_grid(tg, cdiv(w_, 32), cdiv(h, 8), N)) return rc;
  return launch_resident<k_conv1_f23<C>>(tg.ntiles, lds, st, "conv1 (F(2,3) along x)", cost, w, c1, h, w_, tg);
}

static int launch_conv1_ksplit32(const float* cost, const float* w, float* c1, int N, int h, int w_, hipStream_t st) {
  constexpr int C = 32;
  constexpr size_t lds = ((size_t)(C / 4) * group_pitch(plane_pitch16(10 * 18), C / 4) + 12 * 64 * 4) * sizeof(float);
  TileGrid tg;
  if (int rc = make_tile_grid(tg, cdiv(w_, 16), cdiv(h, 8), N)) return rc;
  return launch_resident<k_conv1_ksplit<C>>(tg.ntiles, lds, st, "conv1", cost, w, c1, h, w_, tg);
}

template <int C>
static int launch_conv1_c(const float* cost, const float* w, float* c1, int N, int h, int w_, hipStream_t st) {
  constexpr size_t lds = (size_t)(C / 4) * group_pitch(plane_pitch16(10 * 18), C / 4) * sizeof(float);
  TileGrid tg;
  if (int rc = make_tile_grid(tg, cdiv(w_, 16), cdiv(h, 8), N)) return rc;
  return launch_resident<k_conv1_two_row<C>>(tg.ntiles, lds, st, "conv1", cost, w, c1, h, w_, tg);
}

template <int CA, int CB, int NT>
static int launch_small_pro(const SmallConvArgs& a, const GruPro& pro, int B, hipStream_t st) {
  typedef ConvSmallRole<CA, CB, NT, 1, EPI_LINEAR, 4, 1> Role;
  TileGrid tg;
  if (int rc = make_tile_grid(tg, cdiv(a.wo, 16), cdiv(a.ho, 4), B)) return rc;
  return launch_resident<k_conv_small_pro<CA, CB, NT>>(tg.ntiles, Role::LDS_BYTES, st, "conv_pair (folded)", a, tg, pro);
}

int launch_conv_pair(const float* srcA, int CA, const float* srcB, int CB, const float* wpk, const float* bias, float* out,
                     int cout, int B, int h, int w, hipStream_t st, double* gn_part, int gn_hc, int gn_groups, int* gn_parts,
                     const GruPro* pro) {
  SmallConvArgs a{srcA, srcB, wpk, bias, out, nullptr, h, w, h, w, cout};
  if (gn_parts) *gn_parts = 0;
  const long parts = (long)cdiv(w, 16) * cdiv(h, 4) * 4;
  if (gn_part && gn_parts && gn_epilogue_partials(parts, B)) {
    a.gn_part = gn_part; a.gn_hc = gn_hc; a.gn_groups = gn_groups;
    *gn_parts = (int)parts;
  }
  if (pro) {
    if (CB == 8 && cout <= 16) {
      if (CA == 32) return launch_small_pro<32, 8, 1>(a, *pro, B, st);
      if (CA == 16) return launch_small_pro<16, 8, 1>(a, *pro, B, st);
      if (CA == 8) return launch_small_pro<8, 8, 1>(a, *pro, B, st);
    }
    if (CA == 16 && CB == 16 && cout <= 16) return launch_small_pro<16, 16, 1>(a, *pro, B, st);
    if (CA == 16 && CB == 16 && cout <= 32) return launch_small_pro<16, 16, 2>(a, *pro, B, st);
  }
  if (CB == 8 && cout <= 16) {
    if (CA == 32) return launch_small<32, 8, 1, 1, EPI_LINEAR>(a, B, st, "conv_pair");
    if (CA == 16) return launch_small<16, 8, 1, 1, EPI_LINEAR>(a, B, st, "conv_pair");
    if (CA == 8) return launch_small<8, 8, 1, 1, EPI_LINEAR>(a, B, st, "conv_pair");
  }
  if (CA == 16 && CB == 16 && cout <= 16) return launch_small<16, 16, 1, 1, EPI_LINEAR>(a, B, st, "conv_pair");
  if (CA == 16 && CB == 16 && cout <= 32) return launch_small<16, 16, 2, 1, EPI_LINEAR>(a, B, st, "conv_pair");
  return set_error(-1, "conv3x3_pair: (CA=%d, CB=%d, cout=%d) unsupported: (32|16|8, 8, <=16) or (16, 16, <=32)", CA, CB, cout);
}

bool conv_pair_epilogue_partials(int B, int h, int w) { return gn_epilogue_partials((long)cdiv(w, 16) * cdiv(h, 4) * 4, B); }

int launch_conv1(const float* cost, const float* w, float* c1, int N, int C, int h, int w_, int precision, hipStream_t st) {
  if (precision == PRECISION_BF16X3) return launch_conv1_bf16x3(cost, w, c1, N, C, h, w_, st);
  if (C == 32) return (conv1_f23() & 1) ? launch_conv1_f23_32(cost, w, c1, N, h, w_, st) : launch_conv1_ksplit32(cost, w, c1, N, h, w_, st);
  if (C == 16) return (conv1_f23() & 2) ? launch_conv1_f23_rows<16>(cost, w, c1, N, h, w_, st) : launch_conv1_c<16>(cost, w, c1, N, h, w_, st);
  if (C == 8) return (conv1_f23() & 2) ? launch_conv1_f23_rows<8>(cost, w, c1, N, h, w_, st) : launch_conv1_c<8>(cost, w, c1, N, h, w_, st);
  return set_error(-1, "conv1: C=%d unsupported (8, 16 or 32)", C);
}

int launch_slice_step(const float* c1, const FuseWeights& fw, const StepBuffers& sb, float* vol, int B, int h, int w, int D,
                      int d, int in_up, int precision, hipStream_t st, float** h1_now, float** h2_now) {
  int h2 = h / 2, w2 = w / 2, rc;
  float* h1 = sb.h1;
  float* h2s = sb.h2;
  if (precision == PRECISION_BF16X3) {
    if ((rc = launch_gru_convs_bf16x3(c1, fw, sb, B, h, w, d, &h1, &h2s, st))) return rc;
  } else {
  {
    SmallConvArgs g{c1, sb.h1, fw.gates1, fw.gates1_b, sb.rh1, sb.u1, h, w, h, w, 16};
    if ((gru_wino_mask() & 1) && fw.gates1_w) {
      g.wpk = fw.gates1_w;
      if ((rc = launch_small_wino<8, 8, 1, EPI_GATES>(g, B, st, "gates1 (F(2x2,3x3))"))) return rc;
    } else if ((rc = launch_small<8, 8, 1, 1, EPI_GATES>(g, B, st, "gates1"))) return rc;
    SmallConvArgs c{c1, sb.rh1, fw.cand1, fw.cand1_b, sb.h1, sb.u1, h, w, h, w, 8};
    if ((gru_wino_mask() & 8) && fw.cand1_w) {
      c.wpk = fw.cand1_w;
      if ((rc = launch_small_wino<8, 8, 1, EPI_CAND>(c, B, st, "cand1 (F(2x2,3x3))"))) return rc;
    } else if ((rc = launch_cand1_two_row(c, B, st))) return rc;
  }
  {
    SmallConvArgs a{h1, nullptr, fw.conv2, nullptr, sb.c2, nullptr, h, w, h2, w2, 16};
    if ((rc = launch_small<8, 0, 1, 2, EPI_RELU>(a, B, st, "conv2"))) return rc;
  }
  {
    SmallConvArgs g{sb.c2, sb.h2, fw.gates2, fw.gates2_b, sb.rh2, sb.u2, h2, w2, h2, w2, 32};
    if ((gru_wino_mask() & 2) && fw.gates2_w) {
      g.wpk = fw.gates2_w;
      if ((rc = launch_small_wino<16, 16, 2, EPI_GATES>(g, B, st, "gates2 (F(2x2,3x3))"))) return rc;
    } else if ((rc = launch_small<16, 16, 2, 1, EPI_GATES>(g, B, st, "gates2"))) return rc;
    SmallConvArgs c{sb.c2, sb.rh2, fw.cand2, fw.cand2_b, sb.h2, sb.u2, h2, w2, h2, w2, 16};
    if ((gru_wino_mask() & 4) && fw.cand2_w) {
      c.wpk = fw.cand2_w;
      if ((rc = launch_small_wino<16, 16, 1, EPI_CAND>(c, B, st, "cand2 (F(2x2,3x3))"))) return rc;
    } else if ((rc = launch_small<16, 16, 1, 1, EPI_CAND>(c, B, st, "cand2"))) return rc;
  }
  }
  if (h1_now) *h1_now = h1;
  if (h2_now) *h2_now = h2s;
  DecoderArgs da{h2s, h1, fw.upconv1, fw.upconv1_b, fw.final_w, vol, h, w, D, d};
  TileGrid tg;
  if ((rc = make_tile_grid(tg, cdiv(w, DecoderRole<true>::TCI), cdiv(h, DecoderRole<true>::TRI), B))) return rc;
  constexpr size_t dlds = DecoderRole<true>::LDS_BYTES;
  if (in_up) return launch_resident<k_decoder<true>>(tg.ntiles, dlds, st, "decoder", da, tg);
  return launch_resident<k_decoder<false>>(tg.ntiles, dlds, st, "decoder", da, tg);
}

int launch_soft_argmin(const float* vol, const float* planes, float* depth, float* conf, int B, int D, int h, int w,
                       int in_up, hipStream_t st) {
  size_t total = (size_t)B * (in_up ? 4 : 1) * h * w;
  unsigned nb = (unsigned)((total + 255) / 256);
  if (in_up) hipLaunchKernelGGL((k_soft_argmin<true>), dim3(nb), dim3(256), 0, st, vol, planes, depth, conf, D, h, w, total);
  else hipLaunchKernelGGL((k_soft_argmin<false>), dim3(nb), dim3(256), 0, st, vol, planes, depth, conf, D, h, w, total);
  ADAMVS_CHECK_LAUNCH("soft_argmin");
  return 0;
}

}
```

### ada-mvs_amd/csrc/slice_roles.h

```cpp
#pragma once
#include "common.h"
#include "conv_frag.h"
#include "kernels.h"
#include "persistent.h"

namespace adamvs {

enum { EPI_RELU = 0, EPI_GATES = 1, EPI_CAND = 2, EPI_LINEAR = 3 };

struct SmallConvArgs {
  const float* srcA;
  const float* srcB;
  const float* wpk;
  const float* bias;
  float* dst0;
  float* dst1;
  int hi, wi, ho, wo, cout;
  const float* hin;
  double* gn_part;
  int gn_hc, gn_groups;
};

struct TileRange { int begin, end; };

// ... 623 lines not shown
#pragma unroll
    for (int j = 0; j < NRUN; ++j) {
      const int ys = ys0 + (src[j] & 0xffff), xs = xs0 + (src[j] >> 16);
      const bool ok = ((unsigned)ys < (unsigned)h && (unsigned)xs < (unsigned)w) || (DEC_PAIR && !((rmask >> j) & 1u));
      hreg[j] = buf_load4(r1, ok ? h1off[j] : BUF_OOB);
      in |= ok ? (1u << j) : 0u;
    }
    return in;
  };
  auto store_h2 = [&](const f32x4 (&stage)[NH]) {
#pragma unroll
    for (int k = 0; k < NH; ++k) {
      float* dl = (float*)((char*)lh2 + h2lds[k]);
      f32x4 v = stage[k];
      dl[0] = v.x; dl[HPLANE] = v.y; dl[2 * HPLANE] = v.z; dl[3 * HPLANE] = v.w;
    }
  };

  int t = tr.begin + wg;
  if (t >= tr.end) return;
  int b, tx, ty;
  tile_coords(tg, t, b, tx, ty);
  f32x4 stage[NH], hreg[NRUN];
  load_h2(stage, b, tx, ty);
  unsigned inside = load_h1(hreg, b, tx, ty);
  wait_vmem_all();
  store_h2(stage);
  __syncthreads();
  for (;;) {
    const int tn = t + nwg;
    const bool more = tn < tr.end;
    int bn = 0, txn = 0, tyn = 0;
    if (more) {
      tile_coords(tg, tn, bn, txn, tyn);
      load_h2(stage, bn, txn, tyn);
    }

    f32x4 sv[NRUN];
#if DEC_PAIR
    {
      auto chain1 = [&](unsigned x0, unsigned x1) {
        f32x4 acc = {0.f, 0.f, 0.f, 0.f};
#pragma unroll
        for (int kc = 0; kc < 4; ++kc) {
          const char* b0 = (const char*)lh2 + x0 + kc * HGP * 4;
          const char* b1 = (const char*)lh2 + x1 + kc * HGP * 4;
          acc = mfma16(P1[0][kc], *(const float*)b0, acc);
          acc = mfma16(P1[1][kc], *(const float*)(b0 + 4), acc);
          acc = mfma16(P1[2][kc], *(const float*)b1, acc);
          acc = mfma16(P1[3][kc], *(const float*)(b1 + 4), acc);
        }
        return acc;
      };
      auto chain0 = [&](unsigned x0, unsigned x1) {
        f32x4 acc = {0.f, 0.f, 0.f, 0.f};
#pragma unroll
        for (int kc = 0; kc < 4; ++kc) {
          acc = mfma16(P0[0][kc], *(const float*)((const char*)lh2 + x0 + kc * HGP * 4), acc);
          acc = mfma16(P0[1][kc], *(const float*)((const char*)lh2 + x1 + kc * HGP * 4), acc);
        }
        return acc;
      };
      sv[0] = chain1(xbyte[0], xbyte1[0]);
      sv[1] = chain0(xbyte[1], xbyte1[1]);
      if (wave < 2) sv[2] = chain1(xbyte[2], xbyte1[2]);
      else sv[2] = chain0(xbyte[2], xbyte1[2]);
    }
#else
    sv[0] = upconv1_class<0, 0, HGP, HCOLS>(wf, lh2, xbyte[0]);
    sv[1] = upconv1_class<0, 1, HGP, HCOLS>(wf, lh2, xbyte[1]);
    sv[2] = upconv1_class<1, 0, HGP, HCOLS>(wf, lh2, xbyte[2]);
    sv[3] = upconv1_class<1, 1, HGP, HCOLS>(wf, lh2, xbyte[3]);
    switch (wave) {
      case 0: sv[4] = upconv1_class<0, 0, HGP, HCOLS>(wf, lh2, xbyte[4]); break;
      case 1: sv[4] = upconv1_class<0, 1, HGP, HCOLS>(wf, lh2, xbyte[4]); break;
      case 2: sv[4] = upconv1_class<1, 0, HGP, HCOLS>(wf, lh2, xbyte[4]); break;
      default: sv[4] = upconv1_class<1, 1, HGP, HCOLS>(wf, lh2, xbyte[4]); break;
    }
#endif
#pragma unroll
    for (int j = 0; j < NRUN; ++j) drain(sv[j]);
    const bool all_in = __builtin_amdgcn_readfirstlane(__builtin_amdgcn_ballot_w64(inside != ALL_IN) == 0) != 0;
    if (DEC_PAIR || q < 2) {
#pragma unroll
      for (int j = 0; j < NRUN; ++j) {
        f32x4 v = sv[j] + bup + hreg[j];
        v.x = fmaxf(v.x, 0.f); v.y = fmaxf(v.y, 0.f); v.z = fmaxf(v.z, 0.f); v.w = fmaxf(v.w, 0.f);
        sv[j] = v;
      }
      if (!all_in) {
#pragma unroll
        for (int j = 0; j < NRUN; ++j)
          if (!((inside >> j) & 1u)) sv[j] = f32x4{0.f, 0.f, 0.f, 0.f};
      }
#pragma unroll
      for (int j = 0; j < NRUN; ++j)
        if (!DEC_PAIR || ((rmask >> j) & 1u)) *(f32x4*)((char*)ls + sbyte[j]) = sv[j];
    }
    unsigned inside_n = ALL_IN;
    if (more) inside_n = load_h1(hreg, bn, txn, tyn);
    __syncthreads();

    const int y0 = ty * TRI, x0 = tx * TCI;
    const bool full = y0 + TRI <= h && x0 + TCI <= w;
    unsigned oo = ooff;
    if (!full) oo = (y0 + pi < h && x0 + pj < w) ? ooff : BUF_OOB;
    const char* sp = (const char*)ls + qbyte;
    cfloat* wfin = wfin0;
    asm volatile("" : "+s"(wfin));
    auto spix = [&](int dy, int dx, f32x2 (&v)[4]) {
      const f32x4 lo = *(const f32x4*)(sp + (dy * SC + dx) * SPX * 4), hi = *(const f32x4*)(sp + (dy * SC + dx) * SPX * 4 + 16);
      v[0] = f32x2{lo.x, lo.y}; v[1] = f32x2{lo.z, lo.w}; v[2] = f32x2{hi.x, hi.y}; v[3] = f32x2{hi.z, hi.w};
    };
    auto tap = [&](f32x2& acc, int t9, const f32x2 (&v)[4]) {
#pragma unroll
      for (int c2 = 0; c2 < 4; ++c2) acc += *(const f32x2 __attribute__((address_space(4)))*)(wfin + t9 * 8 + 2 * c2) * v[c2];
    };
    const float bf = wfin[72];
    if (IN_UP) {
      const buf_rsrc ro = make_rsrc((char*)a.vol + ((((long)b * a.D + a.d) * Ho + 2 * y0) * (long)Wo + 2 * x0) * 4);
      f32x2 s00[4], s01[4], s10[4], s11[4];
      spix(0, 0, s00); spix(0, 1, s01); spix(1, 0, s10); spix(1, 1, s11);
      f32x2 o00 = {bf, 0.f}, o01 = {bf, 0.f}, o10 = {bf, 0.f}, o11 = {bf, 0.f};
      tap(o00, 4, s00);
      tap(o01, 5, s00); tap(o01, 3, s01);
      tap(o10, 7, s00); tap(o10, 1, s10);
      tap(o11, 8, s00); tap(o11, 6, s01); tap(o11, 2, s10); tap(o11, 0, s11);
      __builtin_amdgcn_raw_buffer_store_b64(u32x2{__float_as_uint(o00.x + o00.y), __float_as_uint(o01.x + o01.y)}, ro, oo, 0, 0);
      __builtin_amdgcn_raw_buffer_store_b64(u32x2{__float_as_uint(o10.x + o10.y), __float_as_uint(o11.x + o11.y)}, ro,
                                            oo == BUF_OOB ? BUF_OOB : oo + (unsigned)Wo * 4u, 0, 0);
    } else {
      const buf_rsrc ro = make_rsrc((char*)a.vol + ((((long)b * a.D + a.d) * Ho + y0) * (long)Wo + x0) * 4);
      f32x2 o = {bf, 0.f};
#pragma unroll
      for (int ky = 0; ky < 3; ++ky)
#pragma unroll
        for (int kx = 0; kx < 3; ++kx) {
          f32x2 v[4];
          spix(ky, kx, v);
          tap(o, ky * 3 + kx, v);
        }
      __builtin_amdgcn_raw_buffer_store_b32(__float_as_uint(o.x + o.y), ro, oo, 0, 0);
    }
    if (!more) break;
    wait_vmem_all();
    __syncthreads();
    store_h2(stage);
    __syncthreads();
    t = tn; b = bn; tx = txn; ty = tyn; inside = inside_n;
  }
  }
};
enum { TR_CAND = 0, TR_BIAS_RELU = 1 };
template <int EPI2>
struct TwoRowPairRole {
  typedef SmallConvArgs Args;
  static constexpr int CA = 8, CB = 8, C = 16, KC = C / 4, G = C / 4, GA = CA / 4, TR = 8, TC = 16, LR = TR + 2, LC = TC + 2;
  static constexpr int NPIX = LR * LC, PLANE = plane_pitch16(NPIX), GP = group_pitch(PLANE, G);
  static constexpr int NA = (NPIX * GA + 255) / 256, NL = 2 * NA;
  static constexpr size_t LDS_BYTES = (size_t)G * GP * sizeof(float);
  static constexpr int TILE_W = TC, TILE_H = TR;
  static int tiles_x(const Args& a) { return cdiv(a.wo, TC); }
  static int tiles_y(const Args& a) { return cdiv(a.ho, TR); }

  static __device__ __forceinline__ void run(const Args& a, const TileGrid& tg, TileRange tr, int wg, int nwg, float* lds) {
  const int tid = threadIdx.x, lane = tid & 63, wave = __builtin_amdgcn_readfirstlane(tid >> 6);
  const int p = lane & 15, q = lane >> 4;
  const int h = a.hi, w = a.wi;
  float wf[12][KC];
#pragma unroll
  for (int t = 0; t < 12; ++t)
#pragma unroll
    for (int kc = 0; kc < KC; ++kc) wf[t][kc] = a.wpk[(t * KC + kc) * 64 + lane];
  const f32x4 bias = *(const f32x4*)(a.bias + 4 * (q & 1));

  unsigned goff[NL], lbyte[NL];
  int rc[NL];
#pragma unroll
  for (int k = 0; k < NL; ++k) {
    const bool isA = k < NA;
    const int j = min(tid + (isA ? k : k - NA) * 256, NPIX * GA - 1);
    const int g = j % GA, pp = j / GA, r = pp / LC, c = pp % LC;
    goff[k] = (unsigned)(((r * w + c) * CA + 4 * g) * 4);
    lbyte[k] = (unsigned)((((isA ? 0 : GA) + g) * GP + r * LC + c) * 4);
    rc[k] = r | (c << 16);
    pin(goff[k]); pin(lbyte[k]); pin(rc[k]);
  }
  unsigned xbyte[KC];
#pragma unroll
  for (int kc = 0; kc < KC; ++kc) {
    xbyte[kc] = (unsigned)((kc * GP + q * PLANE + (2 * wave) * LC + p) * 4);
    pin(xbyte[kc]);
  }
  const int orow = 2 * wave + (q >> 1);
  unsigned ooff = (unsigned)(((orow * w + p) * 8 + 4 * (q & 1)) * 4);
  pin(ooff);

  auto load_tile = [&](f32x4 (&stage)[NL], int n, int tx, int ty) {
    const int ix0 = tx * TC - 1, iy0 = ty * TR - 1;
    const long pix0 = ((long)n * h + iy0) * w + ix0;
    const buf_rsrc ra = make_rsrc((const char*)a.srcA + pix0 * (CA * 4));
    const buf_rsrc rb = make_rsrc((const char*)a.srcB + pix0 * (CB * 4));
    if (iy0 >= 0 && ix0 >= 0 && iy0 + LR <= h && ix0 + LC <= w) {
#pragma unroll
      for (int k = 0; k < NL; ++k) stage[k] = buf_load4(k < NA ? ra : rb, goff[k]);
    } else {
#pragma unroll
      for (int k = 0; k < NL; ++k) {
        const int iy = iy0 + (rc[k] & 0xffff), ix = ix0 + (rc[k] >> 16);
        stage[k] = buf_load4(k < NA ? ra : rb, ((unsigned)iy < (unsigned)h && (unsigned)ix < (unsigned)w) ? goff[k] : BUF_OOB);
      }
    }
  };
  auto store_tile = [&](const f32x4 (&stage)[NL]) {
#pragma unroll
    for (int k = 0; k < NL; ++k) {
      float* dl = (float*)((char*)lds + lbyte[k]);
      f32x4 v = stage[k];
      dl[0] = v.x; dl[PLANE] = v.y; dl[2 * PLANE] = v.z; dl[3 * PLANE] = v.w;
    }
  };

  int t = tr.begin + wg;
  if (t >= tr.end) return;
  int n, tx, ty;
  tile_coords(tg, t, n, tx, ty);
  f32x4 stage[NL];
  load_tile(stage, n, tx, ty);
  wait_vmem_all();
  store_tile(stage);
  __syncthreads();
  for (;;) {
    const int y0 = ty * TR, x0 = tx * TC;
    const long opix0 = ((long)n * h + y0) * w + x0;
    const buf_rsrc rh = make_rsrc((char*)a.dst0 + opix0 * 32);
    const buf_rsrc rin = make_rsrc((const char*)(a.hin ? a.hin : a.dst0) + opix0 * 32);
    const buf_rsrc ru = make_rsrc((const char*)a.dst1 + opix0 * 32);
    unsigned oo = ooff;
    if (!(y0 + TR <= h && x0 + TC <= w)) oo = (y0 + orow < h && x0 + p < w) ? ooff : BUF_OOB;
    f32x4 pre_u = {0.f, 0.f, 0.f, 0.f}, pre_h = pre_u;
    if (EPI2 == TR_CAND) { pre_u = buf_load4(ru, oo); pre_h = buf_load4(rin, oo); }
    const int tn = t + nwg;
    const bool more = tn < tr.end;
    int nn = 0, txn = 0, tyn = 0;
    if (more) {
      tile_coords(tg, tn, nn, txn, tyn);
      load_tile(stage, nn, txn, tyn);
    }
    f32x4 acc = {0.f, 0.f, 0.f, 0.f};
#pragma unroll
    for (int rr = 0; rr < 4; ++rr)
#pragma unroll
      for (int kx = 0; kx < 3; ++kx)
#pragma unroll
        for (int kc = 0; kc < KC; ++kc)
          acc = mfma16(wf[rr * 3 + kx][kc], *(const float*)((const char*)lds + xbyte[kc] + (rr * LC + kx) * 4), acc);
    drain(acc);

    wait_vmem_all();
    __syncthreads();
    if (more) store_tile(stage);

    const f32x4 v = acc + bias;
    if (EPI2 == TR_CAND) {
      const f32x4 cnd = {tanh_fast(v.x), tanh_fast(v.y), tanh_fast(v.z), tanh_fast(v.w)};
      buf_store4(rh, oo, pre_u * pre_h + (1.0f - pre_u) * cnd);
    } else {
      buf_store4(rh, oo, f32x4{fmaxf(v.x, 0.f), fmaxf(v.y, 0.f), fmaxf(v.z, 0.f), fmaxf(v.w, 0.f)});
    }
    if (!more) break;
    __syncthreads();
    t = tn; n = nn; tx = txn; ty = tyn;
  }
  }
};
typedef TwoRowPairRole<TR_CAND> Cand1TwoRowRole;

}
```

### ada-mvs_amd/csrc/slice_roles_wino.h

```cpp
#pragma once
#include "slice_roles.h"

#ifndef WINO_GRU_EXP
#define WINO_GRU_EXP 0
#endif

namespace adamvs {

typedef float f32x2w __attribute__((ext_vector_type(2)));
typedef unsigned u32x2w __attribute__((ext_vector_type(2)));

#ifndef WINO_GRU_IL
#define WINO_GRU_IL 1
#endif
#ifndef WINO_GRU_RPR2
#define WINO_GRU_RPR2 1
#endif

template <int CA, int CB, int NT, int EPI>
struct ConvWinoRole {
  typedef SmallConvArgs Args;
  static_assert(EPI == EPI_GATES || EPI == EPI_CAND, "the GRU epilogues");
  static constexpr int CIN = CA + CB, KC = CIN / 4, G = KC, GA = CA / 4, GB = CB / 4, HC = CB;
  static constexpr int TR = 8, TC = 32, LR = TR + 2, LC = TC + 2, NPIX = LR * LC;
  static constexpr int PLANE = plane_pitch16(NPIX), GP = group_pitch(PLANE, G);
  static_assert((PLANE % 2) == 0 && (GP % 2) == 0 && (LC % 2) == 0, "8-byte aligned patch reads");
  static constexpr int NA = (NPIX * GA + 255) / 256, NB = (NPIX * GB + 255) / 256, NL = NA + NB;
  static constexpr int Z0 = (G * GP + 3) & ~3;
  static constexpr int ZBUF = 4 * 2 * NT * 64 * 4;
  static constexpr int RPR = (WINO_GRU_RPR2 && EPI == EPI_CAND && NT == 1 && KC == 8) ? 2 : 1;
  static constexpr size_t LDS_BYTES = (size_t)(Z0 + 2 * RPR * ZBUF) * sizeof(float);
  static constexpr int TILE_W = TC, TILE_H = TR;
  static int tiles_x(const Args& a) { return cdiv(a.wo, TC); }
  static int tiles_y(const Args& a) { return cdiv(a.ho, TR); }

  static __device__ __forceinline__ void run(const Args& a, const TileGrid& tg, TileRange tr, int wg, int nwg, float* lds) {
  const int tid = threadIdx.x, lane = tid & 63, wave = __builtin_amdgcn_readfirstlane(tid >> 6);
  const int p = lane & 15, q = lane >> 4;

  constexpr bool IL = WINO_GRU_IL && EPI == EPI_GATES && NT == 1 && HC == 8;
  const int row_of_lane = IL ? ((lane & 2) ? 8 + 2 * ((lane & 15) >> 2) + (lane & 1) : 2 * ((lane & 15) >> 2) + (lane & 1)) : (lane & 15);
  const int src_lane = (lane & 48) | row_of_lane;
  float uf[NT][4][KC];
#pragma unroll
  for (int nt = 0; nt < NT; ++nt)
#pragma unroll
    for (int j = 0; j < 4; ++j)
#pragma unroll
      for (int kc = 0; kc < KC; ++kc) uf[nt][j][kc] = a.wpk[((((nt * 4 + wave) * 4 + j) * KC) + kc) * 64 + src_lane];
  constexpr float PRE = EPI == EPI_GATES ? -1.4426950408889634f : 2.8853900817779268f;
  f32x4 bias[NT];
#pragma unroll
  for (int nt = 0; nt < NT; ++nt) {
    const f32x4 b = IL ? f32x4{a.bias[2 * q], a.bias[2 * q + 1], a.bias[8 + 2 * q], a.bias[8 + 2 * q + 1]} : *(const f32x4*)(a.bias + nt * 16 + 4 * q);
    bias[nt] = WINO_GRU_IL ? (wave == 1 ? b * PRE : f32x4{0.f, 0.f, 0.f, 0.f}) : b * PRE;
    if (WINO_GRU_IL) drain(bias[nt]);
  }

  unsigned goff[NL], lbyte[NL];
#pragma unroll
  for (int k = 0; k < NL; ++k) {
    const bool isA = k < NA;
    const int gs = isA ? GA : GB, cs = isA ? CA : CB;
    int j = tid + (isA ? k : k - NA) * 256;
    j = min(j, NPIX * gs - 1);
    const int g = j % gs, pp = j / gs, r = pp / LC, c = pp % LC;
    goff[k] = (unsigned)(((r * a.wi + c) * cs + 4 * g) * 4);
    lbyte[k] = (unsigned)((((isA ? 0 : GA) + g) * GP + r * LC + c) * 4);
    pin(goff[k]); pin(lbyte[k]);
  }
  const int rowA = wave == 0 ? 0 : (wave == 2 ? 2 : 1);
  const int rowB = wave == 3 ? 3 : (wave == 2 ? 1 : 2);
  const float sgn = wave == 1 ? 1.0f : -1.0f;
  const f32x2w sgn2 = {sgn, sgn};
  unsigned pa = (unsigned)((q * PLANE + rowA * LC + 2 * p) * 4), pb = (unsigned)((q * PLANE + rowB * LC + 2 * p) * 4);
  pin(pa); pin(pb);
  const int oa = wave >> 1, ob = wave & 1;
  const float os = oa ? -1.0f : 1.0f;
  const int CO = HC;
  unsigned ooff = (unsigned)(((oa * a.wo + 2 * p + ob) * CO + 4 * q) * 4);
  pin(ooff);
  const unsigned hbyte = IL ? (unsigned)(((GA + (q >> 1)) * GP + 2 * (q & 1) * PLANE + (oa + 1) * LC + 2 * p + ob + 1) * 4)
                            : (unsigned)(((GA + min(q, GB - 1)) * GP + (oa + 1) * LC + 2 * p + ob + 1) * 4);
  unsigned ooff2 = (unsigned)(((oa * a.wo + 2 * p + ob) * CO + 2 * q) * 4);
  if (IL) pin(ooff2);
  float* zl = lds + Z0;

  auto load_tile = [&](f32x4 (&stage)[NL], int b, int tx, int ty) {
    const int ix0 = tx * TC - 1, iy0 = ty * TR - 1;
    const long pix0 = ((long)b * a.hi + iy0) * a.wi + ix0;
    const buf_rsrc ra = make_rsrc((const char*)a.srcA + pix0 * (CA * 4));
    const buf_rsrc rb = make_rsrc((const char*)a.srcB + pix0 * (CB * 4));
    if (iy0 >= 0 && ix0 >= 0 && iy0 + LR <= a.hi && ix0 + LC <= a.wi) {
#pragma unroll
      for (int k = 0; k < NL; ++k) stage[k] = buf_load4(k < NA ? ra : rb, goff[k]);
    } else {
#pragma unroll
      for (int k = 0; k < NL; ++k) {
        const bool isA = k < NA;
        const int gs = isA ? GA : GB;
        const int pp = min(tid + (isA ? k : k - NA) * 256, NPIX * gs - 1) / gs;
        const int iy = iy0 + pp / LC, ix = ix0 + pp % LC;
        stage[k] = buf_load4(isA ? ra : rb, ((unsigned)iy < (unsigned)a.hi && (unsigned)ix < (unsigned)a.wi) ? goff[k] : BUF_OOB);
      }
    }
  };
  auto store_tile = [&](const f32x4 (&stage)[NL]) {
#pragma unroll
    for (int k = 0; k < NL; ++k) {
      float* dl = (float*)((char*)lds + lbyte[k]);
      const f32x4 v = stage[k];
      dl[0] = v.x; dl[PLANE] = v.y; dl[2 * PLANE] = v.z; dl[3 * PLANE] = v.w;
    }
  };

  int t = tr.begin + wg;
  if (t >= tr.end) return;
  int b, tx, ty;
  tile_coords(tg, t, b, tx, ty);
  f32x4 stage[NL];
  load_tile(stage, b, tx, ty);
  wait_vmem_all();
  store_tile(stage);
  __syncthreads();
  for (;;) {
    const int oy0 = ty * TR, ox0 = tx * TC;
    const long opix0 = ((long)b * a.ho + oy0) * a.wo + ox0;
    const buf_rsrc r0 = make_rsrc((char*)a.dst0 + opix0 * (CO * 4));
    const buf_rsrc r1 = make_rsrc((char*)a.dst1 + opix0 * (CO * 4));
    const buf_rsrc rin = make_rsrc((const char*)(a.hin ? a.hin : a.dst0) + opix0 * (CO * 4));
    const bool full = oy0 + TR <= a.ho && ox0 + TC <= a.wo;
    f32x4 pre_u[EPI == EPI_CAND ? 4 : 1][NT], pre_h[EPI == EPI_CAND ? 4 : 1][NT];
    if (EPI == EPI_CAND) {
#pragma unroll
      for (int r = 0; r < 4; ++r) {
        unsigned o = ooff + (unsigned)(2 * r * a.wo * CO * 4);
        if (!full && !(oy0 + 2 * r + oa < a.ho && ox0 + 2 * p + ob < a.wo)) o = BUF_OOB;
#pragma unroll
        for (int nt = 0; nt < NT; ++nt) {
          const unsigned on = (o != BUF_OOB && nt * 16 + 4 * q < HC) ? o + nt * 64 : BUF_OOB;
          pre_u[EPI == EPI_CAND ? r : 0][nt] = buf_load4(r1, on);
          pre_h[EPI == EPI_CAND ? r : 0][nt] = buf_load4(rin, on);
        }
      }
    }
    const int tn = t + nwg;
    const bool more = tn < tr.end;
    int bn = 0, txn = 0, tyn = 0;
    if (more) {
      tile_coords(tg, tn, bn, txn, tyn);
      load_tile(stage, bn, txn, tyn);
    }

#pragma unroll
    for (int rd = 0; rd < 4 / RPR; ++rd) {
      f32x4 m[RPR][NT][4];
#pragma unroll
      for (int rr = 0; rr < RPR; ++rr)
#pragma unroll
        for (int nt = 0; nt < NT; ++nt)
#pragma unroll
          for (int j = 0; j < 4; ++j) m[rr][nt][j] = (WINO_GRU_IL && j == 1) ? bias[nt] : f32x4{0.f, 0.f, 0.f, 0.f};
#pragma unroll
      for (int kc = 0; kc < KC; ++kc)
#pragma unroll
        for (int rr = 0; rr < RPR; ++rr) {
          const int tr4 = rd * RPR + rr;
          const int off = (kc * GP + 2 * tr4 * LC) * 4;
          const f32x2w a01 = *(const f32x2w*)((const char*)lds + pa + off), a23 = *(const f32x2w*)((const char*)lds + pa + off + 8);
          const f32x2w b01 = *(const f32x2w*)((const char*)lds + pb + off), b23 = *(const f32x2w*)((const char*)lds + pb + off + 8);
          const f32x2w t01 = __builtin_elementwise_fma(sgn2, b01, a01), t23 = __builtin_elementwise_fma(sgn2, b23, a23);
          const f32x2w v03 = t01 - t23;
          float v0 = v03.x, v3 = v03.y, v1 = t01.y + t23.x, v2 = t23.x - t01.y;
          if (WINO_GRU_EXP & 4) { v0 = a01.x; v1 = a01.y; v2 = b23.x; v3 = b23.y; }
#pragma unroll
          for (int nt = 0; nt < NT; ++nt) {
            m[rr][nt][0] = mfma16(uf[nt][0][kc], v0, m[rr][nt][0]);
            m[rr][nt][1] = mfma16(uf[nt][1][kc], v1, m[rr][nt][1]);
            m[rr][nt][2] = mfma16(uf[nt][2][kc], v2, m[rr][nt][2]);
            m[rr][nt][3] = mfma16(uf[nt][3][kc], v3, m[rr][nt][3]);
          }
        }
#pragma unroll
      for (int rr = 0; rr < RPR; ++rr)
#pragma unroll
        for (int nt = 0; nt < NT; ++nt)
#pragma unroll
          for (int j = 0; j < 4; ++j) drain(m[rr][nt][j]);
      f32x4* zb = (f32x4*)(zl + (rd & 1) * (RPR * ZBUF));
#pragma unroll
      for (int rr = 0; rr < RPR; ++rr)
#pragma unroll
        for (int nt = 0; nt < NT; ++nt) {
          if (WINO_GRU_EXP & 8) break;
          zb[rr * (ZBUF / 4) + ((wave * 2 + 0) * NT + nt) * 64 + lane] = (m[rr][nt][0] + m[rr][nt][1]) + m[rr][nt][2];
          zb[rr * (ZBUF / 4) + ((wave * 2 + 1) * NT + nt) * 64 + lane] = (m[rr][nt][1] - m[rr][nt][2]) - m[rr][nt][3];
        }
      if (!(WINO_GRU_EXP & (1 | 8))) __syncthreads();
#pragma unroll
      for (int rr = 0; rr < RPR; ++rr) {
      const int tr4 = rd * RPR + rr;
      unsigned oo = ooff + (unsigned)(2 * tr4 * a.wo * CO * 4);
      if (!full && !(oy0 + 2 * tr4 + oa < a.ho && ox0 + 2 * p + ob < a.wo)) oo = BUF_OOB;
#pragma unroll
      for (int nt = 0; nt < NT; ++nt) {
        f32x4 z0 = zb[rr * (ZBUF / 4) + (((oa + 0) * 2 + ob) * NT + nt) * 64 + lane];
        f32x4 z1 = zb[rr * (ZBUF / 4) + (((oa + 1) * 2 + ob) * NT + nt) * 64 + lane];
        f32x4 z2 = zb[rr * (ZBUF / 4) + (((oa + 2) * 2 + ob) * NT + nt) * 64 + lane];
        if (WINO_GRU_EXP & 8) { z0 = (m[rr][nt][0] + m[rr][nt][1]) + m[rr][nt][2]; z1 = z0; z2 = (m[rr][nt][1] - m[rr][nt][2]) - m[rr][nt][3]; }
        const f32x4 v = WINO_GRU_IL ? z0 + os * (z1 + z2) : (z0 + os * (z1 + z2)) + bias[nt];
        const int co4 = nt * 16 + 4 * q;
        if (IL) {
          const f32x4 sg = (WINO_GRU_EXP & 2) ? v : f32x4{sigmoid_pre(v.x), sigmoid_pre(v.y), sigmoid_pre(v.z), sigmoid_pre(v.w)};
          const float* hl = (const float*)((const char*)lds + hbyte + 2 * tr4 * LC * 4);
          const float h0 = hl[0], h1 = hl[PLANE];
          unsigned o2 = ooff2 + (unsigned)(2 * tr4 * a.wo * CO * 4);
          if (oo == BUF_OOB) o2 = BUF_OOB;
          __builtin_amdgcn_raw_buffer_store_b64(u32x2w{__float_as_uint(sg.x * h0), __float_as_uint(sg.y * h1)}, r0, o2, 0, 0);
          __builtin_amdgcn_raw_buffer_store_b64(u32x2w{__float_as_uint(sg.z), __float_as_uint(sg.w)}, r1, o2, 0, 0);
        } else if (EPI == EPI_GATES) {
          const f32x4 sg = (WINO_GRU_EXP & 2) ? v : f32x4{sigmoid_pre(v.x), sigmoid_pre(v.y), sigmoid_pre(v.z), sigmoid_pre(v.w)};
          if (co4 < HC) {
            const float* hl = (const float*)((const char*)lds + hbyte + 2 * tr4 * LC * 4);
            const f32x4 hc = {hl[0], hl[PLANE], hl[2 * PLANE], hl[3 * PLANE]};
            buf_store4(r0, oo == BUF_OOB ? BUF_OOB : oo + nt * 64, sg * hc);
          } else if (co4 < 2 * HC) {
            buf_store4(r1, oo == BUF_OOB ? BUF_OOB : oo + (unsigned)((co4 - HC - 4 * q) * 4), sg);
          }
        } else if (co4 < HC) {
          const f32x4 cnd = {tanh_pre(v.x), tanh_pre(v.y), tanh_pre(v.z), tanh_pre(v.w)};
          const f32x4 u4 = pre_u[EPI == EPI_CAND ? tr4 : 0][nt], h4 = pre_h[EPI == EPI_CAND ? tr4 : 0][nt];
          buf_store4(r0, oo == BUF_OOB ? BUF_OOB : oo + nt * 64, gru_blend(u4, h4, cnd));
        }
      }
      }
    }

    wait_vmem_all();
    __syncthreads();
    if (more) store_tile(stage);
    if (!more) break;
    __syncthreads();
    t = tn; b = bn; tx = txn; ty = tyn;
  }
  }
};

}
```

### ada-mvs_amd/packing.py

```python
import os

import torch

BN_EPS = 1e-5

REG_LAYERS = ("conv0", "conv1", "conv2", "conv3", "conv4", "conv5", "conv6", "conv7", "conv9", "conv11", "prob")
REG_TRANSPOSED = ("conv7", "conv9", "conv11")
REG_WINOGRAD = ("conv0", "conv2", "conv4", "conv6", "prob")
WINO_WIDTHS = (64, 128, 192, 256, 384, 512)
REG_WIDTHS = {"fp32": (16, 32, 48, 64, 96, 128, 192, 256, 384, 512), "bf16x3": (32, 64, 96, 128, 192, 256, 384, 512)}
PAD_SCORE = -1e30


def reg_width(d, precision="fp32"):
    for w in REG_WIDTHS[precision]:
        if d <= w:
            return w
    raise ValueError("CostRegNet2D: %d hypotheses (at most %d)" % (d, REG_WIDTHS[precision][-1]))


def _as_cout_cin_tap(w, transposed):
    w = w.detach().to(torch.float32).cpu()
    if transposed:
        w = w.permute(1, 0, 2, 3)
    return w.reshape(w.shape[0], w.shape[1], 9).contiguous()


def split_bf16(x):
    hi = x.to(torch.bfloat16)
    lo = (x - hi.to(torch.float32)).to(torch.bfloat16)
    return hi, lo


def pack_small_conv(w, transposed=False):
    w = _as_cout_cin_tap(w, transposed)
    cout, cin = w.shape[0], w.shape[1]
    assert cin % 4 == 0
    nt = (cout + 15) // 16
    wp = torch.zeros(nt * 16, cin, 9)
    wp[:cout] = w
    return wp.reshape(nt, 16, cin // 4, 4, 9).permute(0, 4, 2, 3, 1).contiguous().reshape(-1)


def pack_conv1_two_row(w):
    w = w.detach().to(torch.float32).cpu()
    cout, cin = w.shape[0], w.shape[1]
    assert cout == 8 and cin % 4 == 0
    wp = torch.zeros(4, 3, 16, cin)
    for rr in range(4):
        if rr <= 2:
            wp[rr, :, :8] = w[:, :, rr, :].permute(2, 0, 1)
        if rr >= 1:
            wp[rr, :, 8:] = w[:, :, rr - 1, :].permute(2, 0, 1)
    return wp.reshape(4, 3, 16, cin // 4, 4).permute(0, 1, 3, 4, 2).contiguous().reshape(-1)


def _pack_rows_bf16x3(wm):
    rows, k = wm.shape
    nt, nkb = rows // 16, (k + 31) // 32
    wp = torch.zeros(rows, nkb * 32)
    wp[:, :k] = wm
    parts = []
    for part in split_bf16(wp):
        parts.append(part.reshape(nt, 16, nkb, 4, 8).permute(0, 2, 3, 1, 4).contiguous())
    frag = torch.stack(parts, 1).contiguous().reshape(-1)
    if frag.numel() % 2:
        frag = torch.cat([frag, torch.zeros(1, dtype=torch.bfloat16)])
    return frag.view(torch.float32)


def pack_small_conv_bf16x3(w):
    w = _as_cout_cin_tap(w, False)
    cout, cin = w.shape[0], w.shape[1]
    assert cin % 8 == 0
    nt = (cout + 15) // 16
    wm = torch.zeros(nt * 16, 9 * cin)
    wm[:cout] = w.permute(0, 2, 1).reshape(cout, 9 * cin)
    return _pack_rows_bf16x3(wm)


def pack_conv1_two_row_bf16x3(w):
    w = w.detach().to(torch.float32).cpu()
    cout, cin = w.shape[0], w.shape[1]
    assert cout == 8 and cin % 8 == 0
    wm = torch.zeros(16, 4, 3, cin)
    for rr in range(4):
        if rr <= 2:
            wm[:8, rr] = w[:, :, rr, :].permute(0, 2, 1)
        if rr >= 1:
            wm[8:, rr] = w[:, :, rr - 1, :].permute(0, 2, 1)
    return _pack_rows_bf16x3(wm.reshape(16, 12 * cin))


def pad_bias(b, n):
    out = torch.zeros(n)
    out[:b.numel()] = b.detach().to(torch.float32).cpu().reshape(-1)
    return out


def pack_reg_layer(w, scale, shift, transposed):
    w = _as_cout_cin_tap(w, transposed) * scale.reshape(-1, 1, 1)
    d = w.shape[0]
    assert w.shape[1] == d and d % 16 == 0, "CostRegNet2D width must be a multiple of 16"
    frag = w.reshape(d // 16, 16, d // 4, 4, 9).permute(4, 2, 0, 3, 1).contiguous().reshape(-1)
    return torch.cat([frag, shift.detach().to(torch.float32).cpu().reshape(-1)])


WINO_G = torch.tensor([[1.0, 0.0, 0.0], [0.5, 0.5, 0.5], [0.5, -0.5, 0.5], [0.0, 0.0, 1.0]], dtype=torch.float64)


def pack_reg_layer_wino(w, scale):
    w = (w.detach().to(torch.float64).cpu() * scale.detach().to(torch.float64).cpu().reshape(-1, 1, 1, 1))
    d = w.shape[0]
    assert w.shape[1] == d and d % 16 == 0
    u = torch.einsum("ik,ockl,jl->ijoc", WINO_G, w, WINO_G).to(torch.float32)
    return u.reshape(4, 4, d // 16, 16, d // 4, 4).permute(4, 0, 2, 5, 3, 1).contiguous().reshape(-1)


def pack_reg_layer_bf16x3(w, scale, shift, transposed):
    w = _as_cout_cin_tap(w, transposed) * scale.reshape(-1, 1, 1)
    d = w.shape[0]
    assert w.shape[1] == d and d % 32 == 0, "bf16x3 CostRegNet2D width must be a multiple of 32"
    halves = []
    for part in split_bf16(w):
        halves.append(part.reshape(d // 16, 16, d // 32, 4, 8, 9).permute(5, 2, 0, 3, 1, 4).contiguous().reshape(-1))
    frag = torch.cat(halves).view(torch.float32)
    assert frag.numel() == 9 * d * d
    return torch.cat([frag, shift.detach().to(torch.float32).cpu().reshape(-1)])


def _pad_square(w, transposed, dr):
    d = w.shape[0]
    if d == dr:
        return w
    out = torch.zeros(dr, dr, 3, 3, dtype=w.dtype)
    out[:d, :d] = w.detach().cpu()
    return out


def pack_cost_reg_net_2d(sd, pre, precision="fp32"):
    pack_layer = pack_reg_layer if precision == "fp32" else pack_reg_layer_bf16x3
    d = sd[pre + "prob.weight"].shape[0]
    dr = reg_width(d, precision)

    def pad_vec(v, fill):
        out = torch.full((dr,), float(fill))
        out[:d] = v.detach().float().cpu()
        return out

    chunks, wino = [], []
    for name in REG_LAYERS:
        if name == "prob":
            w = sd[pre + "prob.weight"]
            scale = torch.ones(w.shape[0])
            shift = sd[pre + "prob.bias"]
            transposed = False
        else:
            transposed = name in REG_TRANSPOSED
            wkey, bnpre = (pre + name + ".0.weight", pre + name + ".1.") if transposed else \
                          (pre + name + ".conv.weight", pre + name + ".bn.")
            w = sd[wkey]
            g = sd[bnpre + "weight"].detach().float().cpu()
            b = sd[bnpre + "bias"].detach().float().cpu()
            mu = sd[bnpre + "running_mean"].detach().float().cpu()
            var = sd[bnpre + "running_var"].detach().float().cpu()
            scale = g / torch.sqrt(var + BN_EPS)
            shift = b - mu * scale
        w = _pad_square(w, transposed, dr)
        scale, shift = pad_vec(scale, 1.0), pad_vec(shift, PAD_SCORE if (name == "prob" and dr > d) else 0.0)
        chunks.append(pack_layer(w, scale, shift, transposed))
        if precision == "fp32" and name in REG_WINOGRAD and dr in WINO_WIDTHS:
            wino.append(pack_reg_layer_wino(w, scale))
    return torch.cat(chunks + wino)


FUSE_FIELDS = ("conv1", "gates1", "gates1_b", "cand1", "cand1_b", "conv2", "gates2", "gates2_b",
               "cand2", "cand2_b", "upconv1", "upconv1_b", "final_w", "gates1_w", "gates2_w", "cand2_w", "cand1_w")


def pack_small_conv_wino(w, scale=1.0):
    w = w.detach().to(torch.float64).cpu() * scale
    cout, cin = w.shape[0], w.shape[1]
    assert cin % 4 == 0
    nt = (cout + 15) // 16
    u = torch.zeros(4, 4, nt * 16, cin, dtype=torch.float32)
    u[:, :, :cout] = torch.einsum("ik,ockl,jl->ijoc", WINO_G, w, WINO_G).to(torch.float32)
    return u.reshape(4, 4, nt, 16, cin // 4, 4).permute(2, 0, 1, 4, 5, 3).contiguous().reshape(-1)


def pack_slice_reg_net(sd, pre, precision="fp32"):
    pack_small, pack_c1 = (pack_small_conv, pack_conv1_two_row) if precision == "fp32" else \
                          (pack_small_conv_bf16x3, pack_conv1_two_row_bf16x3)
    wg1, bg1 = sd[pre + "conv_gru1.conv_gates.0.weight"], sd[pre + "conv_gru1.conv_gates.0.bias"]
    LOG2E = 1.4426950408889634
    gs, cs = (1.0, 1.0) if precision == "fp32" else (-LOG2E, 2.0 * LOG2E)
    scaled = lambda key, s: sd[pre + key].detach().cpu().double().mul(s).float()
    if precision != "fp32":
        wg1, bg1 = scaled("conv_gru1.conv_gates.0.weight", gs), scaled("conv_gru1.conv_gates.0.bias", gs)
        perm = torch.tensor([2 * (m // 4) + (m % 4) if m % 4 < 2 else 8 + 2 * (m // 4) + (m % 4 - 2) for m in range(16)])
        wg1, bg1 = wg1.detach().cpu()[perm], bg1.detach().cpu()[perm]
    parts = {
        "conv1": pack_c1(sd[pre + "conv1.conv.weight"]),
        "gates1": pack_small(wg1),
        "gates1_b": pad_bias(bg1, 16),
        "cand1": (pack_c1 if precision == "fp32" or os.environ.get("ADAMVS_BX3_CAND_TWO_ROW", "1") != "0" else pack_small)(
            scaled("conv_gru1.convc.0.weight", cs)),
# ... 219 lines not shown
```

Before: 658.5 depth maps/s.

## Fuse conv2 into gates1 Winograd kernel and add lagged recurrence schedule

Adds a Gates1Conv2 Winograd role that computes the stride-2 conv2 of the previous level-1 state from the LDS window already loaded for gates1, removing a separate conv2 launch and its reload of h1. A new recurrence schedule (mode 6, lag 1) is chosen by default when the pipelined mode is off, running gates1+conv2, level-2 GRU, decoder and cand1 in a lagged order. It also adds a 32-wide cand1 two-row tile variant that shares load offsets, and moves the gates1 bias into LDS. The cost is more register and LDS pressure per block and a different step dependency structure.

New measurement: 665.6 depth maps/s, median of 6. 1.1% higher.

```diff
diff --git a/ada-mvs_amd/csrc/api.hip b/ada-mvs_amd/csrc/api.hip
--- a/ada-mvs_amd/csrc/api.hip
+++ b/ada-mvs_amd/csrc/api.hip
@@ -262,7 +262,8 @@
   const size_t c1_stride = (size_t)s.B * hw * 8;
   GruStateRing rb{{ws + c.h1[0], ws + c.h1[1], ws + c.h1[2], ws + c.h1[3]}, ws + c.rh1, ws + c.u1, {ws + c.c2[0], ws + c.c2[1]},
                   {ws + c.h2[0], ws + c.h2[1]}, ws + c.rh2, ws + c.u2};
-  const int mode = recurrence_mode(s.precision_fuse, (long)s.B * s.h * s.w);
+  int mode = recurrence_mode(s.precision_fuse, (long)s.B * s.h * s.w);
+  if (mode == 0 && conv2_in_gates1_applies(fw, s.h, s.w, s.precision_fuse)) mode = 6;
   const bool pipelined = mode != 0;
   const int lag = recurrence_lags(mode, s.precision_fuse).dec;
   if (do_rec) {
diff --git a/ada-mvs_amd/csrc/kernels.h b/ada-mvs_amd/csrc/kernels.h
--- a/ada-mvs_amd/csrc/kernels.h
+++ b/ada-mvs_amd/csrc/kernels.h
@@ -25,6 +25,9 @@
   const float* gates1_w; const float* gates2_w; const float* cand2_w; const float* cand1_w;
 };
 int gru_wino_mask();
+enum { GRU_WINO_CONV2_APART = 16, GRU_WINO_CAND1_TILE16 = 32, GRU_WINO_SLOT_A_FUSED = 64 };
+inline bool conv2_in_gates1_enabled() { return !(gru_wino_mask() & GRU_WINO_CONV2_APART); }
+inline bool cand1_tile32_enabled() { return !(gru_wino_mask() & GRU_WINO_CAND1_TILE16); }
 
 struct StepBuffers {
   float* h1; float* rh1; float* u1;
@@ -40,6 +43,10 @@
 RecurLags recurrence_lags(int schedule, int precision);
 int launch_recur_pipeline_step(const GruStateRing& rb, const FuseWeights& fw, int B, int h, int w, int D, int t, const float* c1_t,
                                float* vol_dec, int D_vol, int d_dec, int in_up, int precision, int schedule, hipStream_t st);
+bool conv2_in_gates1_applies(const FuseWeights& fw, int h, int w, int precision);
+int launch_lagged_step(const FuseWeights& fw, int B, int h, int w, int D, int t, const float* c1_t, const float* h1_prev, float* h1_new,
+                       float* rh1, float* u1, float* c2, const float* h2_prev, float* h2_new, float* rh2, float* u2, float* vol_dec, int D_vol,
+                       int d_dec, int in_up, hipStream_t st);
 int launch_soft_argmin_chunk(const float* vol, int vol_D, PlaneSrc planes, int D, int d0, int nd, float* acc, int first, int last,
                              float* depth, float* conf, int B, int h, int w, int in_up, hipStream_t st);
 int sweep_chunk_planes(int D);
diff --git a/ada-mvs_amd/csrc/options.h b/ada-mvs_amd/csrc/options.h
--- a/ada-mvs_amd/csrc/options.h
+++ b/ada-mvs_amd/csrc/options.h
@@ -18,6 +18,8 @@
   X(OPT_CONV1_F23, "conv1_f23", 3)                             \
   X(OPT_FCONV_F23, "fconv_f23", 1)                                \
   X(OPT_GRU_WINO, "gru_wino", 7)                      \
+                                                     \
+                                                                                \
   X(OPT_RECUR_MODE, "recur_mode", -1)
 
 enum Option {
diff --git a/ada-mvs_amd/csrc/recurrence.hip b/ada-mvs_amd/csrc/recurrence.hip
--- a/ada-mvs_amd/csrc/recurrence.hip
+++ b/ada-mvs_amd/csrc/recurrence.hip
@@ -30,6 +30,7 @@
 template <> struct min_blocks<Gru2FusedBx3Role> { static constexpr int value = 2; };
 template <> struct min_blocks<Gru2FusedRole<4>> { static constexpr int value = 2; };
 template <> struct min_blocks<ConvWinoRole<16, 16, 2, EPI_GATES>> { static constexpr int value = 2; };
+template <> struct min_blocks<Gates1Conv2WinoRole> { static constexpr int value = 4; };
 constexpr int imax3(int a, int b, int c) { return a > b ? (a > c ? a : c) : (b > c ? b : c); }
 
 template <class R0, class R1, class R2>
@@ -177,6 +178,7 @@
 typedef ConvSmallRole<16, 16, 2, 1, EPI_GATES> Gates2;
 typedef ConvSmallRole<16, 16, 1, 1, EPI_CAND> Cand2;
 typedef ConvWinoRole<8, 8, 1, EPI_GATES> Gates1W;
+typedef Gates1Conv2WinoRole Gates1Conv2W;
 typedef ConvWinoRole<16, 16, 2, EPI_GATES> Gates2W;
 typedef ConvWinoRole<16, 16, 1, EPI_CAND> Cand2W;
 typedef Gru1FusedRole<4, 2> Gru1S;
@@ -231,6 +233,7 @@
 
 RecurLags recurrence_lags(int schedule, int precision) {
   if (schedule == 5) return RecurLags{2, 3};
+  if (schedule == 6) return RecurLags{1, 1};
   return RecurLags{1, 2};
 }
 
@@ -245,6 +248,9 @@
   auto C2 = [&](int s) { return rb.c2[((s % 2) + 2) % 2]; };
   const RoleCosts& k = role_costs();
   int rc;
+  if (schedule == 6)
+    return launch_lagged_step(fw, B, h, w, D, t, c1_t, H1(t - 1), H1(t), rb.rh1, rb.u1, C2(t - 1), H2(t - 2), H2(t - 1), rb.rh2, rb.u2, vol_dec,
+                              D_vol, d_dec, in_up, st);
   DecoderArgs da{H2(sd), H1(sd), fw.upconv1, fw.upconv1_b, fw.final_w, vol_dec, h, w, D_vol, d_dec};
 
   if (precision == PRECISION_BF16X3) {
@@ -319,7 +325,12 @@
     SmallConvArgs g1w = g1, g2w = g2, c2w = c2;
     g1w.wpk = fw.gates1_w; g2w.wpk = fw.gates2_w; c2w.wpk = fw.cand2_w;
     const float kg1 = 4.f * 0.76f * k.g1, kg2 = 4.f * 0.69f * k.g2, kc2 = 4.f * 0.89f * k.c2;
-    if (l1 || l2)
+    if (l1 && (gru_wino_mask() & GRU_WINO_SLOT_A_FUSED) && !(h & 1) && !(w & 1)) {
+      Gates1Conv2Args gv{g1w, l2 ? C2(s2) : nullptr, fw.conv2};
+      if ((rc = launch_slot<Gates1Conv2W, NopRole, NopRole>(use<Gates1Conv2W>(&gv, kg1), none<NopRole>(), none<NopRole>(), B, st,
+                                                            "recurrence slot A (F(2x2,3x3), conv2 inside)")))
+        return rc;
+    } else if (l1 || l2)
       if ((rc = launch_slot<Gates1W, Conv2, NopRole>(l1 ? use<Gates1W>(&g1w, kg1) : none<Gates1W>(), l2 ? use<Conv2>(&v2, k.v2) : none<Conv2>(),
                                                      none<NopRole>(), B, st, "recurrence slot A (F(2x2,3x3))")))
         return rc;
diff --git a/ada-mvs_amd/csrc/slice_red.hip b/ada-mvs_amd/csrc/slice_red.hip
--- a/ada-mvs_amd/csrc/slice_red.hip
+++ b/ada-mvs_amd/csrc/slice_red.hip
@@ -13,6 +13,11 @@
   ConvWinoRole<CA, CB, NT, EPI>::run(a, tg, TileRange{0, tg.ntiles}, blockIdx.x, gridDim.x, lds);
 }
 
+__global__ __launch_bounds__(256, 4) void k_gates1_conv2_wino(Gates1Conv2Args a, TileGrid tg) {
+  extern __shared__ __attribute__((aligned(16))) float lds[];
+  Gates1Conv2WinoRole::run(a, tg, TileRange{0, tg.ntiles}, blockIdx.x, gridDim.x, lds);
+}
+
 template <int CA, int CB, int NT, int STRIDE, int EPI, int TR, int RW>
 __global__ __launch_bounds__(256) void k_conv_small(SmallConvArgs a, TileGrid tg) {
   extern __shared__ __attribute__((aligned(16))) float lds[];
@@ -36,6 +41,10 @@
 __global__ __launch_bounds__(256) void k_cand1_two_row(SmallConvArgs a, TileGrid tg) {
   extern __shared__ __attribute__((aligned(16))) float lds[];
   Cand1TwoRowRole::run(a, tg, TileRange{0, tg.ntiles}, blockIdx.x, gridDim.x, lds);
+}
+__global__ __launch_bounds__(256, 4) void k_cand1_two_row32(SmallConvArgs a, TileGrid tg) {
+  extern __shared__ __attribute__((aligned(16))) float lds[];
+  Cand1TwoRowRole32::run(a, tg, TileRange{0, tg.ntiles}, blockIdx.x, gridDim.x, lds);
 }
 
 
@@ -211,6 +220,11 @@
 
 
 static int launch_cand1_two_row(const SmallConvArgs& a, int B, hipStream_t st) {
+  if (cand1_tile32_enabled()) {
+    TileGrid tg;
+    if (int rc = make_tile_grid(tg, Cand1TwoRowRole32::tiles_x(a), Cand1TwoRowRole32::tiles_y(a), B)) return rc;
+    return launch_resident<k_cand1_two_row32>(tg.ntiles, Cand1TwoRowRole32::LDS_BYTES, st, "cand1 (two-row, 8 x 32)", a, tg);
+  }
   constexpr int G = 4;
   constexpr size_t lds = (size_t)G * group_pitch(plane_pitch16(10 * 18), G) * sizeof(float);
   TileGrid tg;
@@ -701,6 +715,68 @@
   return set_error(-1, "conv1: C=%d unsupported (8, 16 or 32)", C);
 }
 
+bool conv2_in_gates1_applies(const FuseWeights& fw, int h, int w, int precision) {
+  return precision == PRECISION_FP32 && conv2_in_gates1_enabled() && (gru_wino_mask() & 1) && fw.gates1_w && !(h & 1) && !(w & 1);
+}
+
+static int launch_cand1(const FuseWeights& fw, const float* c1, float* rh1, float* u1, float* h1_new, const float* h1_prev, int B, int h, int w,
+                        hipStream_t st) {
+  SmallConvArgs c{c1, rh1, fw.cand1, fw.cand1_b, h1_new, u1, h, w, h, w, 8, h1_prev == h1_new ? nullptr : h1_prev};
+  if ((gru_wino_mask() & 8) && fw.cand1_w) {
+    c.wpk = fw.cand1_w;
+    return launch_small_wino<8, 8, 1, EPI_CAND>(c, B, st, "cand1 (F(2x2,3x3))");
+  }
+  return launch_cand1_two_row(c, B, st);
+}
+
+static int launch_decoder(const FuseWeights& fw, const float* h2s, const float* h1, float* vol, int B, int h, int w, int D, int d, int in_up,
+                          hipStream_t st) {
+  DecoderArgs da{h2s, h1, fw.upconv1, fw.upconv1_b, fw.final_w, vol, h, w, D, d};
+  TileGrid tg;
+  if (int rc = make_tile_grid(tg, cdiv(w, DecoderRole<true>::TCI), cdiv(h, DecoderRole<true>::TRI), B)) return rc;
+  constexpr size_t dlds = DecoderRole<true>::LDS_BYTES;
+  if (in_up) return launch_resident<k_decoder<true>>(tg.ntiles, dlds, st, "decoder", da, tg);
+  return launch_resident<k_decoder<false>>(tg.ntiles, dlds, st, "decoder", da, tg);
+}
+
+static int launch_level2(const FuseWeights& fw, float* c2, const float* h2_prev, float* h2_new, float* rh2, float* u2, int B, int h, int w,
+                         hipStream_t st) {
+  const int h2 = h / 2, w2 = w / 2;
+  int rc;
+  SmallConvArgs g{c2, h2_prev, fw.gates2, fw.gates2_b, rh2, u2, h2, w2, h2, w2, 32};
+  if ((gru_wino_mask() & 2) && fw.gates2_w) {
+    g.wpk = fw.gates2_w;
+    if ((rc = launch_small_wino<16, 16, 2, EPI_GATES>(g, B, st, "gates2 (F(2x2,3x3))"))) return rc;
+  } else if ((rc = launch_small<16, 16, 2, 1, EPI_GATES>(g, B, st, "gates2"))) return rc;
+  SmallConvArgs c{c2, rh2, fw.cand2, fw.cand2_b, h2_new, u2, h2, w2, h2, w2, 16, h2_prev == h2_new ? nullptr : h2_prev};
+  if ((gru_wino_mask() & 4) && fw.cand2_w) {
+    c.wpk = fw.cand2_w;
+    return launch_small_wino<16, 16, 1, EPI_CAND>(c, B, st, "cand2 (F(2x2,3x3))");
+  }
+  return launch_small<16, 16, 1, 1, EPI_CAND>(c, B, st, "cand2");
+}
+
+int launch_lagged_step(const FuseWeights& fw, int B, int h, int w, int D, int t, const float* c1_t, const float* h1_prev, float* h1_new,
+                       float* rh1, float* u1, float* c2, const float* h2_prev, float* h2_new, float* rh2, float* u2, float* vol_dec, int D_vol,
+                       int d_dec, int in_up, hipStream_t st) {
+  const int h2 = h / 2, w2 = w / 2;
+  const bool l1 = t < D, l2 = t >= 1 && t <= D;
+  int rc;
+  if (l1) {
+    Gates1Conv2Args a{SmallConvArgs{c1_t, h1_prev, fw.gates1_w, fw.gates1_b, rh1, u1, h, w, h, w, 16}, l2 ? c2 : nullptr, fw.conv2};
+    TileGrid tg;
+    if ((rc = make_tile_grid(tg, Gates1Conv2WinoRole::tiles_x(a), Gates1Conv2WinoRole::tiles_y(a), B))) return rc;
+    if ((rc = launch_resident<k_gates1_conv2_wino>(tg.ntiles, Gates1Conv2WinoRole::LDS_BYTES, st, "gates1 + conv2 (F(2x2,3x3))", a, tg))) return rc;
+  } else if (l2) {
+    SmallConvArgs a{h1_prev, nullptr, fw.conv2, nullptr, c2, nullptr, h, w, h2, w2, 16};
+    if ((rc = launch_small<8, 0, 1, 2, EPI_RELU>(a, B, st, "conv2"))) return rc;
+  }
+  if (l2 && (rc = launch_level2(fw, c2, h2_prev, h2_new, rh2, u2, B, h, w, st))) return rc;
+  if (l2 && (rc = launch_decoder(fw, h2_new, h1_prev, vol_dec, B, h, w, D_vol, d_dec, in_up, st))) return rc;
+  if (l1 && (rc = launch_cand1(fw, c1_t, rh1, u1, h1_new, h1_prev, B, h, w, st))) return rc;
+  return 0;
+}
+
 int launch_slice_step(const float* c1, const FuseWeights& fw, const StepBuffers& sb, float* vol, int B, int h, int w, int D,
                       int d, int in_up, int precision, hipStream_t st, float** h1_now, float** h2_now) {
   int h2 = h / 2, w2 = w / 2, rc;
@@ -715,37 +791,17 @@
       g.wpk = fw.gates1_w;
       if ((rc = launch_small_wino<8, 8, 1, EPI_GATES>(g, B, st, "gates1 (F(2x2,3x3))"))) return rc;
     } else if ((rc = launch_small<8, 8, 1, 1, EPI_GATES>(g, B, st, "gates1"))) return rc;
-    SmallConvArgs c{c1, sb.rh1, fw.cand1, fw.cand1_b, sb.h1, sb.u1, h, w, h, w, 8};
-    if ((gru_wino_mask() & 8) && fw.cand1_w) {
-      c.wpk = fw.cand1_w;
-      if ((rc = launch_small_wino<8, 8, 1, EPI_CAND>(c, B, st, "cand1 (F(2x2,3x3))"))) return rc;
-    } else if ((rc = launch_cand1_two_row(c, B, st))) return rc;
+    if ((rc = launch_cand1(fw, c1, sb.rh1, sb.u1, sb.h1, sb.h1, B, h, w, st))) return rc;
   }
   {
     SmallConvArgs a{h1, nullptr, fw.conv2, nullptr, sb.c2, nullptr, h, w, h2, w2, 16};
     if ((rc = launch_small<8, 0, 1, 2, EPI_RELU>(a, B, st, "conv2"))) return rc;
   }
-  {
-    SmallConvArgs g{sb.c2, sb.h2, fw.gates2, fw.gates2_b, sb.rh2, sb.u2, h2, w2, h2, w2, 32};
-    if ((gru_wino_mask() & 2) && fw.gates2_w) {
-      g.wpk = fw.gates2_w;
-      if ((rc = launch_small_wino<16, 16, 2, EPI_GATES>(g, B, st, "gates2 (F(2x2,3x3))"))) return rc;
-    } else if ((rc = launch_small<16, 16, 2, 1, EPI_GATES>(g, B, st, "gates2"))) return rc;
-    SmallConvArgs c{sb.c2, sb.rh2, fw.cand2, fw.cand2_b, sb.h2, sb.u2, h2, w2, h2, w2, 16};
-    if ((gru_wino_mask() & 4) && fw.cand2_w) {
-      c.wpk = fw.cand2_w;
-      if ((rc = launch_small_wino<16, 16, 1, EPI_CAND>(c, B, st, "cand2 (F(2x2,3x3))"))) return rc;
-    } else if ((rc = launch_small<16, 16, 1, 1, EPI_CAND>(c, B, st, "cand2"))) return rc;
-  }
+  if ((rc = launch_level2(fw, sb.c2, sb.h2, sb.h2, sb.rh2, sb.u2, B, h, w, st))) return rc;
   }
   if (h1_now) *h1_now = h1;
   if (h2_now) *h2_now = h2s;
-  DecoderArgs da{h2s, h1, fw.upconv1, fw.upconv1_b, fw.final_w, vol, h, w, D, d};
-  TileGrid tg;
-  if ((rc = make_tile_grid(tg, cdiv(w, DecoderRole<true>::TCI), cdiv(h, DecoderRole<true>::TRI), B))) return rc;
-  constexpr size_t dlds = DecoderRole<true>::LDS_BYTES;
-  if (in_up) return launch_resident<k_decoder<true>>(tg.ntiles, dlds, st, "decoder", da, tg);
-  return launch_resident<k_decoder<false>>(tg.ntiles, dlds, st, "decoder", da, tg);
+  return launch_decoder(fw, h2s, h1, vol, B, h, w, D, d, in_up, st);
 }
 
 int launch_soft_argmin(const float* vol, const float* planes, float* depth, float* conf, int B, int D, int h, int w,
diff --git a/ada-mvs_amd/csrc/slice_roles.h b/ada-mvs_amd/csrc/slice_roles.h
--- a/ada-mvs_amd/csrc/slice_roles.h
+++ b/ada-mvs_amd/csrc/slice_roles.h
@@ -799,13 +799,13 @@
   }
 };
 enum { TR_CAND = 0, TR_BIAS_RELU = 1 };
-template <int EPI2>
+template <int EPI2, int RW = 1>
 struct TwoRowPairRole {
   typedef SmallConvArgs Args;
-  static constexpr int CA = 8, CB = 8, C = 16, KC = C / 4, G = C / 4, GA = CA / 4, TR = 8, TC = 16, LR = TR + 2, LC = TC + 2;
+  static constexpr int CA = 8, CB = 8, C = 16, KC = C / 4, G = C / 4, GA = CA / 4, TR = 8, TC = 16 * RW, LR = TR + 2, LC = TC + 2;
   static constexpr int NPIX = LR * LC, PLANE = plane_pitch16(NPIX), GP = group_pitch(PLANE, G);
   static constexpr int NA = (NPIX * GA + 255) / 256, NL = 2 * NA;
-  static constexpr size_t LDS_BYTES = (size_t)G * GP * sizeof(float);
+  static constexpr size_t LDS_BYTES = (size_t)(G * GP + (RW > 1 ? 8 : 0)) * sizeof(float);
   static constexpr int TILE_W = TC, TILE_H = TR;
   static int tiles_x(const Args& a) { return cdiv(a.wo, TC); }
   static int tiles_y(const Args& a) { return cdiv(a.ho, TR); }
@@ -814,28 +814,34 @@
   const int tid = threadIdx.x, lane = tid & 63, wave = __builtin_amdgcn_readfirstlane(tid >> 6);
   const int p = lane & 15, q = lane >> 4;
   const int h = a.hi, w = a.wi;
+  const bool lower = p < 8;
   float wf[12][KC];
 #pragma unroll
-  for (int t = 0; t < 12; ++t)
-#pragma unroll
-    for (int kc = 0; kc < KC; ++kc) wf[t][kc] = a.wpk[(t * KC + kc) * 64 + lane];
-  const f32x4 bias = *(const f32x4*)(a.bias + 4 * (q & 1));
-
+  for (int t = 0; t < (RW > 1 ? 9 : 12); ++t)
+#pragma unroll
+    for (int kc = 0; kc < KC; ++kc) wf[t][kc] = a.wpk[(((RW > 1 && t < 3 && !lower) ? t + 9 : t) * KC + kc) * 64 + lane];
+  f32x4 bias = {0.f, 0.f, 0.f, 0.f};
+  if (RW == 1) bias = *(const f32x4*)(a.bias + 4 * (q & 1));
+  else if (tid < 8) lds[G * GP + tid] = a.bias[tid];
+
+  constexpr bool SHARE = RW > 1;
+  constexpr int NI = SHARE ? NA : NL, NX = SHARE ? 1 : KC;
   unsigned goff[NL], lbyte[NL];
   int rc[NL];
 #pragma unroll
-  for (int k = 0; k < NL; ++k) {
+  for (int k = 0; k < NI; ++k) {
     const bool isA = k < NA;
     const int j = min(tid + (isA ? k : k - NA) * 256, NPIX * GA - 1);
     const int g = j % GA, pp = j / GA, r = pp / LC, c = pp % LC;
     goff[k] = (unsigned)(((r * w + c) * CA + 4 * g) * 4);
     lbyte[k] = (unsigned)((((isA ? 0 : GA) + g) * GP + r * LC + c) * 4);
     rc[k] = r | (c << 16);
-    pin(goff[k]); pin(lbyte[k]); pin(rc[k]);
+    pin(goff[k]); pin(lbyte[k]);
+    if (!SHARE) pin(rc[k]);
   }
   unsigned xbyte[KC];
 #pragma unroll
-  for (int kc = 0; kc < KC; ++kc) {
+  for (int kc = 0; kc < NX; ++kc) {
     xbyte[kc] = (unsigned)((kc * GP + q * PLANE + (2 * wave) * LC + p) * 4);
     pin(xbyte[kc]);
   }
@@ -850,19 +856,20 @@
     const buf_rsrc rb = make_rsrc((const char*)a.srcB + pix0 * (CB * 4));
     if (iy0 >= 0 && ix0 >= 0 && iy0 + LR <= h && ix0 + LC <= w) {
 #pragma unroll
-      for (int k = 0; k < NL; ++k) stage[k] = buf_load4(k < NA ? ra : rb, goff[k]);
+      for (int k = 0; k < NL; ++k) stage[k] = buf_load4(k < NA ? ra : rb, goff[k % NI]);
     } else {
 #pragma unroll
       for (int k = 0; k < NL; ++k) {
-        const int iy = iy0 + (rc[k] & 0xffff), ix = ix0 + (rc[k] >> 16);
-        stage[k] = buf_load4(k < NA ? ra : rb, ((unsigned)iy < (unsigned)h && (unsigned)ix < (unsigned)w) ? goff[k] : BUF_OOB);
+        const int pp = min(tid + (k % NA) * 256, NPIX * GA - 1) / GA;
+        const int iy = iy0 + (SHARE ? pp / LC : rc[k] & 0xffff), ix = ix0 + (SHARE ? pp % LC : rc[k] >> 16);
+        stage[k] = buf_load4(k < NA ? ra : rb, ((unsigned)iy < (unsigned)h && (unsigned)ix < (unsigned)w) ? goff[k % NI] : BUF_OOB);
       }
     }
   };
   auto store_tile = [&](const f32x4 (&stage)[NL]) {
 #pragma unroll
     for (int k = 0; k < NL; ++k) {
-      float* dl = (float*)((char*)lds + lbyte[k]);
+      float* dl = (float*)((char*)lds + lbyte[k % NI] + (SHARE && k >= NA ? GA * GP * 4 : 0));
       f32x4 v = stage[k];
       dl[0] = v.x; dl[PLANE] = v.y; dl[2 * PLANE] = v.z; dl[3 * PLANE] = v.w;
     }
@@ -883,10 +890,15 @@
     const buf_rsrc rh = make_rsrc((char*)a.dst0 + opix0 * 32);
     const buf_rsrc rin = make_rsrc((const char*)(a.hin ? a.hin : a.dst0) + opix0 * 32);
     const buf_rsrc ru = make_rsrc((const char*)a.dst1 + opix0 * 32);
-    unsigned oo = ooff;
-    if (!(y0 + TR <= h && x0 + TC <= w)) oo = (y0 + orow < h && x0 + p < w) ? ooff : BUF_OOB;
-    f32x4 pre_u = {0.f, 0.f, 0.f, 0.f}, pre_h = pre_u;
-    if (EPI2 == TR_CAND) { pre_u = buf_load4(ru, oo); pre_h = buf_load4(rin, oo); }
+    unsigned oo[RW];
+    f32x4 pre_u[RW], pre_h[RW];
+#pragma unroll
+    for (int j = 0; j < RW; ++j) {
+      oo[j] = ooff + (unsigned)(j * 16 * 32);
+      if (!(y0 + TR <= h && x0 + TC <= w)) oo[j] = (y0 + orow < h && x0 + 16 * j + p < w) ? oo[j] : BUF_OOB;
+      pre_u[j] = pre_h[j] = f32x4{0.f, 0.f, 0.f, 0.f};
+      if (EPI2 == TR_CAND) { pre_u[j] = buf_load4(ru, oo[j]); pre_h[j] = buf_load4(rin, oo[j]); }
+    }
     const int tn = t + nwg;
     const bool more = tn < tr.end;
     int nn = 0, txn = 0, tyn = 0;
@@ -894,26 +906,37 @@
       tile_coords(tg, tn, nn, txn, tyn);
       load_tile(stage, nn, txn, tyn);
     }
-    f32x4 acc = {0.f, 0.f, 0.f, 0.f};
+    f32x4 acc[RW];
+#pragma unroll
+    for (int j = 0; j < RW; ++j) acc[j] = f32x4{0.f, 0.f, 0.f, 0.f};
+    float zero = 0.f;
+    if (RW > 1) pin(zero);
 #pragma unroll
     for (int rr = 0; rr < 4; ++rr)
 #pragma unroll
       for (int kx = 0; kx < 3; ++kx)
 #pragma unroll
         for (int kc = 0; kc < KC; ++kc)
-          acc = mfma16(wf[rr * 3 + kx][kc], *(const float*)((const char*)lds + xbyte[kc] + (rr * LC + kx) * 4), acc);
-    drain(acc);
+#pragma unroll
+          for (int j = 0; j < RW; ++j)
+            acc[j] = mfma16(RW == 1 ? wf[rr * 3 + kx][kc] : (rr == 0 ? (lower ? wf[kx][kc] : zero) : (rr == 3 ? (lower ? zero : wf[kx][kc]) : wf[rr * 3 + kx][kc])),
+                            *(const float*)((const char*)lds + xbyte[kc % NX] + ((SHARE ? kc * GP : 0) + rr * LC + kx + 16 * j) * 4), acc[j]);
+#pragma unroll
+    for (int j = 0; j < RW; ++j) drain(acc[j]);
 
     wait_vmem_all();
     __syncthreads();
     if (more) store_tile(stage);
 
-    const f32x4 v = acc + bias;
-    if (EPI2 == TR_CAND) {
-      const f32x4 cnd = {tanh_fast(v.x), tanh_fast(v.y), tanh_fast(v.z), tanh_fast(v.w)};
-      buf_store4(rh, oo, pre_u * pre_h + (1.0f - pre_u) * cnd);
-    } else {
-      buf_store4(rh, oo, f32x4{fmaxf(v.x, 0.f), fmaxf(v.y, 0.f), fmaxf(v.z, 0.f), fmaxf(v.w, 0.f)});
+#pragma unroll
+    for (int j = 0; j < RW; ++j) {
+      const f32x4 v = acc[j] + (RW == 1 ? bias : *(const f32x4*)(lds + G * GP + 4 * (q & 1)));
+      if (EPI2 == TR_CAND) {
+        const f32x4 cnd = {tanh_fast(v.x), tanh_fast(v.y), tanh_fast(v.z), tanh_fast(v.w)};
+        buf_store4(rh, oo[j], pre_u[j] * pre_h[j] + (1.0f - pre_u[j]) * cnd);
+      } else {
+        buf_store4(rh, oo[j], f32x4{fmaxf(v.x, 0.f), fmaxf(v.y, 0.f), fmaxf(v.z, 0.f), fmaxf(v.w, 0.f)});
+      }
     }
     if (!more) break;
     __syncthreads();
@@ -922,5 +945,6 @@
   }
 };
 typedef TwoRowPairRole<TR_CAND> Cand1TwoRowRole;
+typedef TwoRowPairRole<TR_CAND, 2> Cand1TwoRowRole32;
 
 }
diff --git a/ada-mvs_amd/csrc/slice_roles_wino.h b/ada-mvs_amd/csrc/slice_roles_wino.h
--- a/ada-mvs_amd/csrc/slice_roles_wino.h
+++ b/ada-mvs_amd/csrc/slice_roles_wino.h
@@ -30,11 +30,19 @@
   static constexpr int ZBUF = 4 * 2 * NT * 64 * 4;
   static constexpr int RPR = (WINO_GRU_RPR2 && EPI == EPI_CAND && NT == 1 && KC == 8) ? 2 : 1;
   static constexpr size_t LDS_BYTES = (size_t)(Z0 + 2 * RPR * ZBUF) * sizeof(float);
+  static constexpr int BL0 = Z0 + 2 * RPR * ZBUF;
   static constexpr int TILE_W = TC, TILE_H = TR;
   static int tiles_x(const Args& a) { return cdiv(a.wo, TC); }
   static int tiles_y(const Args& a) { return cdiv(a.ho, TR); }
 
   static __device__ __forceinline__ void run(const Args& a, const TileGrid& tg, TileRange tr, int wg, int nwg, float* lds) {
+    run_impl<false>(a, tg, tr, wg, nwg, lds, nullptr, nullptr);
+  }
+
+  template <bool CONV2>
+  static __device__ __forceinline__ void run_impl(const Args& a, const TileGrid& tg, TileRange tr, int wg, int nwg, float* lds, float* c2,
+                                                  const float* c2w) {
+  static_assert(!CONV2 || (EPI == EPI_GATES && CA == 8 && CB == 8 && NT == 1), "conv2 reads the level-1 state window");
   const int tid = threadIdx.x, lane = tid & 63, wave = __builtin_amdgcn_readfirstlane(tid >> 6);
   const int p = lane & 15, q = lane >> 4;
 
@@ -49,17 +57,26 @@
 #pragma unroll
       for (int kc = 0; kc < KC; ++kc) uf[nt][j][kc] = a.wpk[((((nt * 4 + wave) * 4 + j) * KC) + kc) * 64 + src_lane];
   constexpr float PRE = EPI == EPI_GATES ? -1.4426950408889634f : 2.8853900817779268f;
+  constexpr bool BL = CONV2 && WINO_GRU_IL && IL;
+  unsigned bb = 0u;
+  if (BL) {
+    if (tid < 20) lds[BL0 + tid] = tid < 16 ? a.bias[((tid & 2) ? 8 : 0) + 2 * (tid >> 2) + (tid & 1)] * PRE : 0.f;
+    bb = (unsigned)((BL0 + (wave == 1 ? 4 * q : 16)) * 4);
+    pin(bb);
+  }
   f32x4 bias[NT];
 #pragma unroll
-  for (int nt = 0; nt < NT; ++nt) {
+  for (int nt = 0; nt < NT && !BL; ++nt) {
     const f32x4 b = IL ? f32x4{a.bias[2 * q], a.bias[2 * q + 1], a.bias[8 + 2 * q], a.bias[8 + 2 * q + 1]} : *(const f32x4*)(a.bias + nt * 16 + 4 * q);
     bias[nt] = WINO_GRU_IL ? (wave == 1 ? b * PRE : f32x4{0.f, 0.f, 0.f, 0.f}) : b * PRE;
     if (WINO_GRU_IL) drain(bias[nt]);
   }
 
+  constexpr bool SHARE = CONV2 && CA == CB;
+  constexpr int LSH = SHARE ? GA * GP * 4 : 0;
   unsigned goff[NL], lbyte[NL];
 #pragma unroll
-  for (int k = 0; k < NL; ++k) {
+  for (int k = 0; k < (SHARE ? NA : NL); ++k) {
     const bool isA = k < NA;
     const int gs = isA ? GA : GB, cs = isA ? CA : CB;
     int j = tid + (isA ? k : k - NA) * 256;
@@ -74,17 +91,31 @@
   const float sgn = wave == 1 ? 1.0f : -1.0f;
   const f32x2w sgn2 = {sgn, sgn};
   unsigned pa = (unsigned)((q * PLANE + rowA * LC + 2 * p) * 4), pb = (unsigned)((q * PLANE + rowB * LC + 2 * p) * 4);
-  pin(pa); pin(pb);
+  pin(pa);
+  if (!CONV2) pin(pb);
   const int oa = wave >> 1, ob = wave & 1;
   const float os = oa ? -1.0f : 1.0f;
   const int CO = HC;
   unsigned ooff = (unsigned)(((oa * a.wo + 2 * p + ob) * CO + 4 * q) * 4);
-  pin(ooff);
+  if (!(CONV2 && IL)) pin(ooff);
   const unsigned hbyte = IL ? (unsigned)(((GA + (q >> 1)) * GP + 2 * (q & 1) * PLANE + (oa + 1) * LC + 2 * p + ob + 1) * 4)
                             : (unsigned)(((GA + min(q, GB - 1)) * GP + (oa + 1) * LC + 2 * p + ob + 1) * 4);
   unsigned ooff2 = (unsigned)(((oa * a.wo + 2 * p + ob) * CO + 2 * q) * 4);
   if (IL) pin(ooff2);
   float* zl = lds + Z0;
+  float cw[CONV2 ? 9 : 1][2];
+  unsigned cx = 0u, coff = 0u;
+  const int h2 = a.ho >> 1, w2 = a.wo >> 1;
+  if (CONV2) {
+#pragma unroll
+    for (int t9 = 0; t9 < 9; ++t9)
+#pragma unroll
+      for (int kc = 0; kc < 2; ++kc) cw[CONV2 ? t9 : 0][kc] = c2w[(t9 * 2 + kc) * 64 + lane];
+    cx = (unsigned)((GA * GP + q * PLANE + (2 * wave) * LC + 2 * p) * 4);
+    pin(cx);
+    coff = (unsigned)(((wave * w2 + p) * 16 + 4 * q) * 4);
+    pin(coff);
+  }
 
   auto load_tile = [&](f32x4 (&stage)[NL], int b, int tx, int ty) {
     const int ix0 = tx * TC - 1, iy0 = ty * TR - 1;
@@ -93,7 +124,7 @@
     const buf_rsrc rb = make_rsrc((const char*)a.srcB + pix0 * (CB * 4));
     if (iy0 >= 0 && ix0 >= 0 && iy0 + LR <= a.hi && ix0 + LC <= a.wi) {
 #pragma unroll
-      for (int k = 0; k < NL; ++k) stage[k] = buf_load4(k < NA ? ra : rb, goff[k]);
+      for (int k = 0; k < NL; ++k) stage[k] = buf_load4(k < NA ? ra : rb, goff[SHARE && k >= NA ? k - NA : k]);
     } else {
 #pragma unroll
       for (int k = 0; k < NL; ++k) {
@@ -101,14 +132,14 @@
         const int gs = isA ? GA : GB;
         const int pp = min(tid + (isA ? k : k - NA) * 256, NPIX * gs - 1) / gs;
         const int iy = iy0 + pp / LC, ix = ix0 + pp % LC;
-        stage[k] = buf_load4(isA ? ra : rb, ((unsigned)iy < (unsigned)a.hi && (unsigned)ix < (unsigned)a.wi) ? goff[k] : BUF_OOB);
+        stage[k] = buf_load4(isA ? ra : rb, ((unsigned)iy < (unsigned)a.hi && (unsigned)ix < (unsigned)a.wi) ? goff[SHARE && k >= NA ? k - NA : k] : BUF_OOB);
       }
     }
   };
   auto store_tile = [&](const f32x4 (&stage)[NL]) {
 #pragma unroll
     for (int k = 0; k < NL; ++k) {
-      float* dl = (float*)((char*)lds + lbyte[k]);
+      float* dl = (float*)((char*)lds + lbyte[SHARE && k >= NA ? k - NA : k] + (k >= NA ? LSH : 0));
       const f32x4 v = stage[k];
       dl[0] = v.x; dl[PLANE] = v.y; dl[2 * PLANE] = v.z; dl[3 * PLANE] = v.w;
     }
@@ -151,6 +182,22 @@
       tile_coords(tg, tn, bn, txn, tyn);
       load_tile(stage, bn, txn, tyn);
     }
+    if (CONV2 && c2) {
+      f32x4 acc2 = {0.f, 0.f, 0.f, 0.f};
+#pragma unroll
+      for (int ky = 0; ky < 3; ++ky)
+#pragma unroll
+        for (int kx = 0; kx < 3; ++kx)
+#pragma unroll
+          for (int kc = 0; kc < 2; ++kc)
+            acc2 = mfma16(cw[CONV2 ? ky * 3 + kx : 0][kc], *(const float*)((const char*)lds + cx + (kc * GP + ky * LC + kx) * 4), acc2);
+      drain(acc2);
+      const buf_rsrc rc2 = make_rsrc((char*)c2 + (((long)b * h2 + ty * (TR / 2)) * w2 + tx * (TC / 2)) * 64);
+      const bool in2 = ty * (TR / 2) + wave < h2 && tx * (TC / 2) + p < w2;
+      f32x4 v2 = acc2 + f32x4{0.f, 0.f, 0.f, 0.f};
+      v2.x = fmaxf(v2.x, 0.f); v2.y = fmaxf(v2.y, 0.f); v2.z = fmaxf(v2.z, 0.f); v2.w = fmaxf(v2.w, 0.f);
+      buf_store4(rc2, in2 ? coff : BUF_OOB, v2);
+    }
 
 #pragma unroll
     for (int rd = 0; rd < 4 / RPR; ++rd) {
@@ -160,7 +207,8 @@
 #pragma unroll
         for (int nt = 0; nt < NT; ++nt)
 #pragma unroll
-          for (int j = 0; j < 4; ++j) m[rr][nt][j] = (WINO_GRU_IL && j == 1) ? bias[nt] : f32x4{0.f, 0.f, 0.f, 0.f};
+          for (int j = 0; j < 4; ++j)
+            m[rr][nt][j] = (WINO_GRU_IL && j == 1) ? (BL ? *(const f32x4*)((const char*)lds + bb) : bias[nt]) : f32x4{0.f, 0.f, 0.f, 0.f};
 #pragma unroll
       for (int kc = 0; kc < KC; ++kc)
 #pragma unroll
@@ -200,7 +248,7 @@
 #pragma unroll
       for (int rr = 0; rr < RPR; ++rr) {
       const int tr4 = rd * RPR + rr;
-      unsigned oo = ooff + (unsigned)(2 * tr4 * a.wo * CO * 4);
+      unsigned oo = (CONV2 && IL) ? 0u : ooff + (unsigned)(2 * tr4 * a.wo * CO * 4);
       if (!full && !(oy0 + 2 * tr4 + oa < a.ho && ox0 + 2 * p + ob < a.wo)) oo = BUF_OOB;
 #pragma unroll
       for (int nt = 0; nt < NT; ++nt) {
@@ -246,4 +294,21 @@
   }
 };
 
+struct Gates1Conv2Args {
+  SmallConvArgs g;
+  float* c2;
+  const float* conv2_w;
+};
+struct Gates1Conv2WinoRole {
+  typedef Gates1Conv2Args Args;
+  typedef ConvWinoRole<8, 8, 1, EPI_GATES> Base;
+  static constexpr size_t LDS_BYTES = Base::LDS_BYTES + 80;
+  static constexpr int TILE_W = Base::TILE_W, TILE_H = Base::TILE_H;
+  static int tiles_x(const Args& a) { return Base::tiles_x(a.g); }
+  static int tiles_y(const Args& a) { return Base::tiles_y(a.g); }
+  static __device__ __forceinline__ void run(const Args& a, const TileGrid& tg, TileRange tr, int wg, int nwg, float* lds) {
+    Base::run_impl<true>(a.g, tg, tr, wg, nwg, lds, a.c2, a.conv2_w);
+  }
+};
+
 }
diff --git a/ada-mvs_amd/packing.py b/ada-mvs_amd/packing.py
--- a/ada-mvs_amd/packing.py
+++ b/ada-mvs_amd/packing.py
@@ -52,6 +52,7 @@
             wp[rr, :, :8] = w[:, :, rr, :].permute(2, 0, 1)
         if rr >= 1:
             wp[rr, :, 8:] = w[:, :, rr - 1, :].permute(2, 0, 1)
+    assert not wp[0, :, 8:].any() and not wp[3, :, :8].any()
     return wp.reshape(4, 3, 16, cin // 4, 4).permute(0, 1, 3, 4, 2).contiguous().reshape(-1)
 
 
```
